# eth-cscs/conflux

Measured on NVIDIA B200. Metric: LU GFLOP/s (FP64, (2/3)N^3), higher is better.
Workload: dtype f64

## Files before the change

### conflux_b200/_lib.py

```python
import ctypes
import os

_HERE = os.path.dirname(os.path.abspath(__file__))
LIB_PATH = os.path.join(_HERE, "libconflux_b200.so")
_lib = None

c_double_p = ctypes.POINTER(ctypes.c_double)
c_int_p = ctypes.POINTER(ctypes.c_int)


class ConfluxError(RuntimeError):
    pass


SYMBOLS = [
    "cflx_last_error", "cflx_version", "cflx_device_count", "cflx_get_unique_id", "cflx_comm_create",
    "cflx_comm_barrier", "cflx_comm_destroy", "cflx_host_alloc", "cflx_host_free", "cflx_auto_grid", "cflx_lu_dims", "cflx_init_matrix_host",
    "cflx_lu_create", "cflx_lu_info", "cflx_lu_set_local", "cflx_lu_queue_next_local", "cflx_lu_factor", "cflx_lu_get_factors",
    "cflx_lu_get_permutation", "cflx_lu_residual", "cflx_lu_validate", "cflx_lu_solve", "cflx_lu_launch_count", "cflx_lu_uses_tcgen05", "cflx_lu_set_profiling", "cflx_lu_phase_ms", "cflx_lu_timeline",
    "cflx_lu_set_kernel_timing", "cflx_lu_trailing_stats", "cflx_lu_destroy", "cflx_chol_auto_grid", "cflx_chol_auto_tile", "cflx_chol_dims", "cflx_chol_init_matrix_host",
    "cflx_chol_create", "cflx_chol_info", "cflx_chol_set_local", "cflx_chol_factor", "cflx_chol_get_local", "cflx_chol_validate",
    "cflx_chol_launch_count", "cflx_chol_destroy", "cflx_dbg_gemm_tn", "cflx_dbg_panel", "cflx_dbg_trsm", "cflx_dbg_trsm_left_upper", "cflx_dbg_potrf_tile", "cflx_dbg_push_pivots", "cflx_dbg_ozaki_gemm", "cflx_dbg_umma_peak", "cflx_dbg_last_panel_cycles", "cflx_dbg_fp64_peak", "cflx_dbg_fp64_peak_ex",
]


def _preload_nccl():
    import sys
    for d in sys.path:
        cand = os.path.join(d, "nvidia", "nccl", "lib", "libnccl.so.2")
        if os.path.exists(cand):
            try:
                ctypes.CDLL(cand, mode=ctypes.RTLD_GLOBAL)
                return cand
            except OSError:
                pass
    return None


def lib():
    global _lib
    if _lib is None:
        if not os.path.exists(LIB_PATH):
            raise ConfluxError(
                f"{LIB_PATH} is missing: build it with `python -c 'import __graft_entry__ as g; g.build()'` "
                "(conflux_b200 has no CPU fallback)")
        _preload_nccl()
        L = ctypes.CDLL(LIB_PATH)
        L.cflx_last_error.restype = ctypes.c_char_p
        L.cflx_version.restype = ctypes.c_char_p
        L.cflx_comm_destroy.restype = None
        L.cflx_lu_destroy.restype = None
        L.cflx_comm_destroy.argtypes = [ctypes.c_void_p]
        L.cflx_lu_destroy.argtypes = [ctypes.c_void_p]
        L.cflx_comm_barrier.argtypes = [ctypes.c_void_p]
        L.cflx_comm_create.argtypes = [ctypes.c_int, ctypes.c_int, ctypes.c_void_p, ctypes.c_int,
                                       ctypes.POINTER(ctypes.c_void_p)]
        L.cflx_lu_create.argtypes = [ctypes.c_void_p] + [ctypes.c_int] * 6 + [ctypes.POINTER(ctypes.c_void_p)]
        L.cflx_host_alloc.argtypes = [ctypes.c_size_t, ctypes.POINTER(ctypes.c_void_p)]
        L.cflx_host_free.argtypes = [ctypes.c_void_p]
        L.cflx_lu_info.argtypes = [ctypes.c_void_p, c_int_p]
        L.cflx_lu_set_local.argtypes = [ctypes.c_void_p, ctypes.c_void_p]
        L.cflx_lu_queue_next_local.argtypes = [ctypes.c_void_p, ctypes.c_void_p]
        L.cflx_lu_factor.argtypes = [ctypes.c_void_p, c_double_p]
        L.cflx_lu_get_factors.argtypes = [ctypes.c_void_p, ctypes.c_void_p, ctypes.c_void_p]
        L.cflx_lu_get_permutation.argtypes = [ctypes.c_void_p, ctypes.c_void_p]
        L.cflx_lu_residual.argtypes = [ctypes.c_void_p, c_double_p]
        L.cflx_lu_validate.argtypes = [ctypes.c_void_p, c_double_p, c_double_p]
        L.cflx_lu_solve.argtypes = [ctypes.c_void_p, ctypes.c_int, ctypes.c_void_p, ctypes.c_void_p, c_double_p]
        L.cflx_lu_uses_tcgen05.argtypes = [ctypes.c_void_p]
        L.cflx_lu_launch_count.argtypes = [ctypes.c_void_p, ctypes.POINTER(ctypes.c_int64), ctypes.c_int]
        L.cflx_lu_set_profiling.argtypes = [ctypes.c_void_p, ctypes.c_int]
        L.cflx_lu_phase_ms.argtypes = [ctypes.c_void_p, c_double_p]
        L.cflx_lu_timeline.argtypes = [ctypes.c_void_p, ctypes.c_char_p, ctypes.c_int]
        L.cflx_lu_set_kernel_timing.argtypes = [ctypes.c_void_p, ctypes.c_int]
        L.cflx_lu_trailing_stats.argtypes = [ctypes.c_void_p, c_double_p, c_double_p]
        L.cflx_chol_destroy.restype = None
        L.cflx_chol_destroy.argtypes = [ctypes.c_void_p]
        L.cflx_chol_auto_grid.argtypes = [ctypes.c_int, ctypes.c_int, c_int_p]
        L.cflx_chol_auto_tile.argtypes = [ctypes.c_int] * 3
        L.cflx_chol_dims.argtypes = [ctypes.c_int] * 5 + [c_int_p]
        L.cflx_chol_init_matrix_host.argtypes = [ctypes.c_int] * 6 + [ctypes.c_void_p]
        L.cflx_chol_create.argtypes = [ctypes.c_void_p] + [ctypes.c_int] * 5 + [ctypes.POINTER(ctypes.c_void_p)]
        L.cflx_chol_info.argtypes = [ctypes.c_void_p, c_int_p]
        L.cflx_chol_set_local.argtypes = [ctypes.c_void_p, ctypes.c_void_p]
        L.cflx_chol_factor.argtypes = [ctypes.c_void_p, c_double_p]
        L.cflx_chol_get_local.argtypes = [ctypes.c_void_p, ctypes.c_void_p]
        L.cflx_chol_validate.argtypes = [ctypes.c_void_p, c_double_p, c_double_p]
        L.cflx_chol_launch_count.argtypes = [ctypes.c_void_p, ctypes.POINTER(ctypes.c_int64), ctypes.c_int]
        L.cflx_init_matrix_host.argtypes = [ctypes.c_int] * 8 + [ctypes.c_void_p]
        L.cflx_dbg_gemm_tn.argtypes = [ctypes.c_int] * 3 + [ctypes.c_void_p] * 3 + [ctypes.c_double] * 2 + [
            ctypes.c_void_p, ctypes.c_int, c_double_p]
        L.cflx_dbg_panel.argtypes = [ctypes.c_int, ctypes.c_int] + [ctypes.c_void_p] * 4 + [ctypes.c_int, c_double_p]
        L.cflx_dbg_trsm.argtypes = [ctypes.c_int, ctypes.c_int] + [ctypes.c_void_p] * 5
        L.cflx_dbg_trsm_left_upper.argtypes = [ctypes.c_int, ctypes.c_int] + [ctypes.c_void_p] * 3
        L.cflx_dbg_potrf_tile.argtypes = [ctypes.c_int, ctypes.c_int] + [ctypes.c_void_p] * 4
        L.cflx_dbg_push_pivots.argtypes = [ctypes.c_int, ctypes.c_int, ctypes.c_void_p, ctypes.c_int, ctypes.c_void_p, ctypes.c_int,
                                           ctypes.c_void_p, ctypes.c_void_p]
        L.cflx_dbg_ozaki_gemm.argtypes = [ctypes.c_int] * 3 + [ctypes.c_void_p] * 8 + [ctypes.c_int, c_double_p, c_double_p]
        L.cflx_dbg_umma_peak.argtypes = [ctypes.c_int, ctypes.c_int, c_double_p]
        L.cflx_dbg_fp64_peak.argtypes = [ctypes.c_int, c_double_p]
        L.cflx_dbg_fp64_peak_ex.argtypes = [ctypes.c_int, c_double_p, c_double_p]
        _lib = L
    return _lib


def check(rc, what=""):
    if rc != 0:
        msg = lib().cflx_last_error().decode(errors="replace")
        raise ConfluxError(f"{what} failed with status {rc}: {msg}")
```

### conflux_b200/csrc/dbg.cu

```cuda
#include <vector>

#include "../../include/conflux_b200.h"
#include "common.cuh"
#include "kernels.h"

using namespace cflx;

namespace {
struct DevBuf {
    void* p = nullptr;
    ~DevBuf() { cudaFree(p); }
    int alloc(size_t bytes) {
        CFLX_CUDA(cudaMalloc(&p, bytes + 4096));
        return CFLX_OK;
    }
    template <class T>
    T* as() { return (T*)p; }
};
int check_device() {
    int n = 0;
    if (cudaGetDeviceCount(&n) != cudaSuccess || n == 0) {
        cudaGetLastError();
        set_last_error("no CUDA device visible: conflux_b200 has no CPU fallback");
        return CFLX_ERR_NO_DEVICE;
    }
    return CFLX_OK;
}

__global__ void dmma_peak_kernel(double* out, int iters) {
    double c[16][2];
#pragma unroll
    for (int i = 0; i < 16; ++i) c[i][0] = c[i][1] = 0.0;
    double a = 1.0 + threadIdx.x * 1e-9, b = 1.0 - threadIdx.x * 1e-9;
    for (int it = 0; it < iters; ++it) {
#pragma unroll
        for (int i = 0; i < 16; ++i) dmma884(c[i][0], c[i][1], a, b);
    }
    double s = 0;
#pragma unroll
    for (int i = 0; i < 16; ++i) s += c[i][0] + c[i][1];
    out[blockIdx.x * blockDim.x + threadIdx.x] = s;
}
__global__ void dfma_peak_kernel(double* out, int iters) {
    double c[16];
#pragma unroll
    for (int i = 0; i < 16; ++i) c[i] = i;
    double a = 1.0 + threadIdx.x * 1e-9, b = 1e-9;
    for (int it = 0; it < iters; ++it) {
#pragma unroll
        for (int i = 0; i < 16; ++i) c[i] = fma(c[i], a, b);
    }
    double s = 0;
#pragma unroll
    for (int i = 0; i < 16; ++i) s += c[i];
    out[blockIdx.x * blockDim.x + threadIdx.x] = s;
}
}

static long long g_panel_cycles[8] = {0};

extern "C" {

int cflx_dbg_last_panel_cycles(long long* out8) {
    for (int i = 0; i < 8; ++i) out8[i] = g_panel_cycles[i];
    return CFLX_OK;
}

int cflx_dbg_fp64_peak_ex(int which, double* burst_out, double* sustained_out) {
    CFLX_TRY(check_device());
    int dev = 0, sms = 0;
    CFLX_CUDA(cudaGetDevice(&dev));
    CFLX_CUDA(cudaDeviceGetAttribute(&sms, cudaDevAttrMultiProcessorCount, dev));
    const int threads = 256, blocks = sms * 4;
    DevBuf out;
    CFLX_TRY(out.alloc(sizeof(double) * threads * blocks));
    cudaEvent_t e0, e1;
    CFLX_CUDA(cudaEventCreate(&e0));
    CFLX_CUDA(cudaEventCreate(&e1));
    auto run = [&](int iters, double* tf) -> int {
        CFLX_CUDA(cudaEventRecord(e0));
        if (which == 0) dmma_peak_kernel<<<blocks, threads>>>(out.as<double>(), iters);
        else dfma_peak_kernel<<<blocks, threads>>>(out.as<double>(), iters);
        CFLX_CUDA(cudaEventRecord(e1));
        CFLX_CUDA(cudaEventSynchronize(e1));
        float ms = 0;
        CFLX_CUDA(cudaEventElapsedTime(&ms, e0, e1));
        const double flop = which == 0 ? (double)blocks * (threads / 32) * iters * 16 * 512.0
                                       : (double)blocks * threads * iters * 16 * 2.0;
        *tf = flop / (ms * 1e-3) / 1e12;
        return CFLX_OK;
    };
    double burst = 0, tf = 0;
    for (int rep = 0; rep < 4; ++rep) {
        CFLX_TRY(run(1024, &tf));
        if (rep > 0 && tf > burst) burst = tf;
    }
    double sustained = 0;
    CFLX_TRY(run(262144, &sustained));
    cudaEventDestroy(e0);
    cudaEventDestroy(e1);
    if (burst_out) *burst_out = burst;
    if (sustained_out) *sustained_out = sustained;
    return CFLX_OK;
}
int cflx_dbg_fp64_peak(int which, double* tflops_out) { return cflx_dbg_fp64_peak_ex(which, tflops_out, nullptr); }

int cflx_dbg_gemm_tn(int M, int N, int K, const double* AT, const double* B, const double* C, double alpha, double beta,
                     double* D, int reps, double* ms_out) {
    CFLX_TRY(check_device());
    if (M <= 0 || N <= 0 || K <= 0) return CFLX_ERR_ARG;
    const int64_t ldat = round_up(M, 2), ldb = round_up(N, 2), ldc = ldb;
    DevBuf dA, dB, dC, dD;
    CFLX_TRY(dA.alloc(sizeof(double) * K * ldat));
    CFLX_TRY(dB.alloc(sizeof(double) * K * ldb));
    CFLX_TRY(dC.alloc(sizeof(double) * M * ldc));
    CFLX_TRY(dD.alloc(sizeof(double) * M * ldc));
    CFLX_CUDA(cudaMemset(dA.p, 0, sizeof(double) * K * ldat));
    CFLX_CUDA(cudaMemset(dB.p, 0, sizeof(double) * K * ldb));
    CFLX_CUDA(cudaMemcpy2D(dA.p, ldat * 8, AT, (size_t)M * 8, (size_t)M * 8, K, cudaMemcpyHostToDevice));
    CFLX_CUDA(cudaMemcpy2D(dB.p, ldb * 8, B, (size_t)N * 8, (size_t)N * 8, K, cudaMemcpyHostToDevice));
    if (C) CFLX_CUDA(cudaMemcpy2D(dC.p, ldc * 8, C, (size_t)N * 8, (size_t)N * 8, M, cudaMemcpyHostToDevice));
    else CFLX_CUDA(cudaMemset(dC.p, 0, sizeof(double) * M * ldc));
    GemmArgs g{};
    g.M = M; g.N = (int)ldb; g.K = K;
    g.AT = dA.as<double>(); g.ldat = ldat;
    g.B = dB.as<double>(); g.ldb = ldb;
    g.C = dC.as<double>(); g.ldc = ldc;
    g.D = dD.as<double>(); g.ldd = ldc;
    g.alpha = alpha; g.beta = beta;
    cudaEvent_t e0, e1;
    CFLX_CUDA(cudaEventCreate(&e0));
    CFLX_CUDA(cudaEventCreate(&e1));
    if (reps < 1) reps = 1;
    CFLX_TRY(launch_gemm_tn(g, 0));
    CFLX_CUDA(cudaEventRecord(e0));
    for (int r = 0; r < reps; ++r) CFLX_TRY(launch_gemm_tn(g, 0));
    CFLX_CUDA(cudaEventRecord(e1));
    CFLX_CUDA(cudaEventSynchronize(e1));
    float ms = 0;
    CFLX_CUDA(cudaEventElapsedTime(&ms, e0, e1));
    if (ms_out) *ms_out = ms / reps;
    cudaEventDestroy(e0);
    cudaEventDestroy(e1);
    if (D) CFLX_CUDA(cudaMemcpy2D(D, (size_t)N * 8, dD.p, ldc * 8, (size_t)N * 8, M, cudaMemcpyDeviceToHost));
    CFLX_CUDA(cudaDeviceSynchronize());
    return CFLX_OK;
}

int cflx_dbg_panel(int n, int v, const double* panel, int* perm_out, double* A00_out, double* LU_out, int reps,
                   double* ms_out) {
    CFLX_TRY(check_device());
    if (n < 0 || v <= 0) return CFLX_ERR_ARG;
    const int64_t ld = std::max<int64_t>(2, round_up(n, 2));
    std::vector<double> WT((size_t)v * ld, 0.0);
    for (int r = 0; r < n; ++r)
        for (int c = 0; c < v; ++c) WT[(size_t)c * ld + r] = panel[(size_t)r * v + c];
    DevBuf dW, dW0, dA00, dA00T, dperm;
    CFLX_TRY(dW.alloc(sizeof(double) * v * ld));
    CFLX_TRY(dW0.alloc(sizeof(double) * v * ld));
    CFLX_TRY(dA00.alloc(sizeof(double) * v * v));
    CFLX_TRY(dA00T.alloc(sizeof(double) * v * v));
    CFLX_TRY(dperm.alloc(sizeof(int) * 2 * v));
    CFLX_CUDA(cudaMemcpy(dW0.p, WT.data(), sizeof(double) * v * ld, cudaMemcpyHostToDevice));
    CFLX_CUDA(cudaMemset(dA00.p, 0, sizeof(double) * v * v));
    PanelWorkspace ws{};
    CFLX_TRY(panel_workspace_create(&ws));
    cudaEvent_t e0, e1;
    CFLX_CUDA(cudaEventCreate(&e0));
    CFLX_CUDA(cudaEventCreate(&e1));
    if (reps < 1) reps = 1;
    float total = 0;
    int nb = 0, rc = CFLX_OK;
    for (int r = 0; r < reps + 1 && rc == CFLX_OK; ++r) {
        cudaMemcpyAsync(dW.p, dW0.p, sizeof(double) * v * ld, cudaMemcpyDeviceToDevice, 0);
        cudaEventRecord(e0);
        rc = launch_panel_getrf_a00(dW.as<double>(), ld, n, v, dperm.as<int>(), dA00.as<double>(), &nb, &ws, 0);
        cudaEventRecord(e1);
        if (cudaEventSynchronize(e1) != cudaSuccess) rc = CFLX_ERR_CUDA;
        float ms = 0;
        cudaEventElapsedTime(&ms, e0, e1);
        if (r > 0) total += ms;
    }
    cudaEventDestroy(e0);
    cudaEventDestroy(e1);
    if (rc == CFLX_OK && n >= v)
        rc = launch_gather_a00(dW.as<double>(), ld, dperm.as<int>(), v, nb, dA00.as<double>(), dA00T.as<double>(), 0);
    cudaMemcpy(g_panel_cycles, ws.dbg, sizeof(g_panel_cycles), cudaMemcpyDeviceToHost);
    panel_workspace_destroy(&ws);
    if (rc != CFLX_OK) {
        if (rc == CFLX_ERR_CUDA) set_last_error("panel kernel failed: %s", cudaGetErrorString(cudaGetLastError()));
        return rc;
    }
    if (ms_out) *ms_out = total / reps;
    if (perm_out) CFLX_CUDA(cudaMemcpy(perm_out, dperm.p, sizeof(int) * v, cudaMemcpyDeviceToHost));
    if (A00_out) CFLX_CUDA(cudaMemcpy(A00_out, dA00.p, sizeof(double) * v * v, cudaMemcpyDeviceToHost));
    if (LU_out) {
        CFLX_CUDA(cudaMemcpy(WT.data(), dW.p, sizeof(double) * v * ld, cudaMemcpyDeviceToHost));
        for (int r = 0; r < n; ++r)
            for (int c = 0; c < v; ++c) LU_out[(size_t)r * v + c] = WT[(size_t)c * ld + r];
    }
    CFLX_CUDA(cudaDeviceSynchronize());
    return CFLX_OK;
}

int cflx_dbg_trsm(int n, int v, const double* A00, const double* B, double* X_out, const double* R, double* Y_out) {
    CFLX_TRY(check_device());
    if (n <= 0 || v <= 0 || v % 4 != 0) return CFLX_ERR_ARG;
    int nb = 0;
    for (int c : {128, 64, 32, 16, 8, 4})
        if (!nb && v % c == 0) nb = c;
    if (nb == 0) return CFLX_ERR_UNSUPPORTED;
    const int64_t ld = round_up(n, 2);
    std::vector<double> A00T((size_t)v * v), BT((size_t)v * ld, 0.0), RT((size_t)v * ld, 0.0);
    for (int i = 0; i < v; ++i)
        for (int j = 0; j < v; ++j) A00T[(size_t)j * v + i] = A00[(size_t)i * v + j];
    DevBuf dA, dAT, dUinv, dLinvT, dP, dL, dR, dU;
    CFLX_TRY(dA.alloc(8 * (size_t)v * v)); CFLX_TRY(dAT.alloc(8 * (size_t)v * v));
    CFLX_TRY(dUinv.alloc(8 * (size_t)v * v)); CFLX_TRY(dLinvT.alloc(8 * (size_t)v * v));
    CFLX_TRY(dP.alloc(8 * (size_t)v * ld)); CFLX_TRY(dL.alloc(8 * (size_t)v * ld));
    CFLX_TRY(dR.alloc(8 * (size_t)v * ld)); CFLX_TRY(dU.alloc(8 * (size_t)v * ld));
    CFLX_CUDA(cudaMemcpy(dA.p, A00, 8 * (size_t)v * v, cudaMemcpyHostToDevice));
    CFLX_CUDA(cudaMemcpy(dAT.p, A00T.data(), 8 * (size_t)v * v, cudaMemcpyHostToDevice));
    CFLX_TRY(launch_diag_inverses(dA.as<double>(), v, nb, dUinv.as<double>(), dLinvT.as<double>(), 0));
    if (B && X_out) {
        for (int r = 0; r < n; ++r)
            for (int c = 0; c < v; ++c) BT[(size_t)c * ld + r] = B[(size_t)r * v + c];
        CFLX_CUDA(cudaMemcpy(dP.p, BT.data(), 8 * (size_t)v * ld, cudaMemcpyHostToDevice));
        CFLX_CUDA(cudaMemset(dL.p, 0, 8 * (size_t)v * ld));
        CFLX_TRY(trsm_right_upper_T(dA.as<double>(), dUinv.as<double>(), v, nb, dP.as<double>(), dL.as<double>(), ld, n, 0));
        CFLX_CUDA(cudaMemcpy(BT.data(), dL.p, 8 * (size_t)v * ld, cudaMemcpyDeviceToHost));
        for (int r = 0; r < n; ++r)
            for (int c = 0; c < v; ++c) X_out[(size_t)r * v + c] = BT[(size_t)c * ld + r];
    }
    if (R && Y_out) {
        for (int i = 0; i < v; ++i)
            for (int c = 0; c < n; ++c) RT[(size_t)i * ld + c] = R[(size_t)i * n + c];
        CFLX_CUDA(cudaMemcpy(dR.p, RT.data(), 8 * (size_t)v * ld, cudaMemcpyHostToDevice));
        CFLX_CUDA(cudaMemset(dU.p, 0, 8 * (size_t)v * ld));
        CFLX_TRY(trsm_left_lower_unit(dAT.as<double>(), dLinvT.as<double>(), v, nb, dR.as<double>(), dU.as<double>(), ld,
                                      (int)ld, 0));
        CFLX_CUDA(cudaMemcpy(RT.data(), dU.p, 8 * (size_t)v * ld, cudaMemcpyDeviceToHost));
        for (int i = 0; i < v; ++i)
            for (int c = 0; c < n; ++c) Y_out[(size_t)i * n + c] = RT[(size_t)i * ld + c];
    }
    CFLX_CUDA(cudaDeviceSynchronize());
    return CFLX_OK;
}

int cflx_dbg_trsm_left_upper(int v, int n, const double* A00, const double* R, double* X_out) {
    CFLX_TRY(check_device());
    if (n <= 0 || v <= 0 || v % 4 != 0 || !A00 || !R || !X_out) return CFLX_ERR_ARG;
    int nb = 0;
    for (int c : {128, 64, 32, 16, 8, 4})
        if (!nb && v % c == 0) nb = c;
    if (nb == 0) return CFLX_ERR_UNSUPPORTED;
    const int64_t ld = round_up(n, 2);
    std::vector<double> A00T((size_t)v * v), RT((size_t)v * ld, 0.0);
    for (int i = 0; i < v; ++i)
        for (int j = 0; j < v; ++j) A00T[(size_t)j * v + i] = A00[(size_t)i * v + j];
    for (int i = 0; i < v; ++i)
        for (int c = 0; c < n; ++c) RT[(size_t)i * ld + c] = R[(size_t)i * n + c];
    DevBuf dA, dAT, dUinvT, dLinvT, dR, dX;
    CFLX_TRY(dA.alloc(8 * (size_t)v * v)); CFLX_TRY(dAT.alloc(8 * (size_t)v * v));
    CFLX_TRY(dUinvT.alloc(8 * (size_t)v * v)); CFLX_TRY(dLinvT.alloc(8 * (size_t)v * v));
    CFLX_TRY(dR.alloc(8 * (size_t)v * ld)); CFLX_TRY(dX.alloc(8 * (size_t)v * ld));
    CFLX_CUDA(cudaMemcpy(dA.p, A00, 8 * (size_t)v * v, cudaMemcpyHostToDevice));
    CFLX_CUDA(cudaMemcpy(dAT.p, A00T.data(), 8 * (size_t)v * v, cudaMemcpyHostToDevice));
    CFLX_CUDA(cudaMemcpy(dR.p, RT.data(), 8 * (size_t)v * ld, cudaMemcpyHostToDevice));
    CFLX_CUDA(cudaMemset(dX.p, 0, 8 * (size_t)v * ld));
    CFLX_TRY(launch_diag_inverses(dA.as<double>(), v, nb, dUinvT.as<double>(), dLinvT.as<double>(), 0, true));
    CFLX_TRY(trsm_left_upper(dAT.as<double>(), dUinvT.as<double>(), v, nb, dR.as<double>(), dX.as<double>(), ld, (int)ld, 0));
    CFLX_CUDA(cudaMemcpy(RT.data(), dX.p, 8 * (size_t)v * ld, cudaMemcpyDeviceToHost));
    for (int i = 0; i < v; ++i)
        for (int c = 0; c < n; ++c) X_out[(size_t)i * n + c] = RT[(size_t)i * ld + c];
    CFLX_CUDA(cudaDeviceSynchronize());
    return CFLX_OK;
}

int cflx_dbg_push_pivots(int n_rows, int n_cols, double* A_inout, int npiv, const int* pivot_rows, int fnpr, int* gri_out,
                         double* a01_out) {
    CFLX_TRY(check_device());
    if (n_rows <= 0 || n_cols <= 0 || (n_cols & 1) || npiv < 0 || npiv > n_rows - fnpr || fnpr < 0) return CFLX_ERR_ARG;
    if (npiv == 0) {
        if (gri_out) for (int i = 0; i < n_rows; ++i) gri_out[i] = i;
        return CFLX_OK;
    }
    const int v = npiv;
    DevBuf dA, dtmp, da01, dplan, dgp, dgri, dgrit, digri;
    CFLX_TRY(dA.alloc(8 * (size_t)n_rows * n_cols));
    CFLX_TRY(dtmp.alloc(8 * (size_t)v * n_cols));
    CFLX_TRY(da01.alloc(8 * (size_t)v * n_cols));
    CFLX_TRY(dplan.alloc(sizeof(int) * (6 * (size_t)v + 8 + n_rows)));
    CFLX_TRY(dgp.alloc(sizeof(int) * v));
    CFLX_TRY(dgri.alloc(sizeof(int) * n_rows));
    CFLX_TRY(dgrit.alloc(sizeof(int) * n_rows));
    CFLX_TRY(digri.alloc(sizeof(int) * n_rows));
    CFLX_CUDA(cudaMemcpy(dA.p, A_inout, 8 * (size_t)n_rows * n_cols, cudaMemcpyHostToDevice));
    CFLX_CUDA(cudaMemcpy(dgp.p, pivot_rows, sizeof(int) * v, cudaMemcpyHostToDevice));
    MovePlan plan{};
    int* pm = dplan.as<int>();
    plan.npiv = pm; plan.nel = pm + 4; pm += 8;
    plan.cur_piv = pm; pm += v;
    plan.order = pm; pm += v;
    plan.slot2piv = pm; pm += v;
    plan.early = pm; pm += v;
    plan.late = pm; pm += 2 * v;
    plan.rowsrc = pm;
    CFLX_TRY(launch_iota_gri(dgri.as<int>(), digri.as<int>(), n_rows, n_rows, 1, 0, 0));
    CFLX_TRY(launch_plan_moves(dgp.as<int>(), v, 1, 0, fnpr, n_rows, digri.as<int>(), plan, 0));
    CFLX_TRY(launch_push_phase1(dA.as<double>(), n_cols, n_cols, 0, plan, v, dtmp.as<double>(), da01.as<double>(), n_cols, 0, 0));
    CFLX_TRY(launch_push_phase2(dA.as<double>(), n_cols, n_cols, 0, plan, v, 0));
    CFLX_TRY(launch_push_phase3(dA.as<double>(), n_cols, n_cols, 0, fnpr, plan, v, dtmp.as<double>(), 0));
    CFLX_TRY(launch_update_gri(dgri.as<int>(), dgrit.as<int>(), digri.as<int>(), plan.rowsrc, fnpr, n_rows, n_rows, 1, 0));
    CFLX_CUDA(cudaMemcpy(A_inout, dA.p, 8 * (size_t)n_rows * n_cols, cudaMemcpyDeviceToHost));
    if (gri_out) CFLX_CUDA(cudaMemcpy(gri_out, dgri.p, sizeof(int) * n_rows, cudaMemcpyDeviceToHost));
    if (a01_out) CFLX_CUDA(cudaMemcpy(a01_out, da01.p, 8 * (size_t)v * n_cols, cudaMemcpyDeviceToHost));
    CFLX_CUDA(cudaDeviceSynchronize());
    return CFLX_OK;
}

int cflx_dbg_ozaki_gemm(int M, int N, int K, const double* AT, const double* B, const double* C, double* D,
                        signed char* planesA_out, signed char* planesB_out, int* ea_out, int* eb_out, int reps,
                        double* ms_out, double* split_ms_out) {
    CFLX_TRY(check_device());
    if (M <= 0 || N <= 0 || K <= 0 || (N & 1)) return CFLX_ERR_ARG;
    const int64_t ldat = round_up(M, 2), ldb = N, ldc = N;
    DevBuf dA, dB, dC, dC0;
    CFLX_TRY(dA.alloc(sizeof(double) * K * ldat));
    CFLX_TRY(dB.alloc(sizeof(double) * K * ldb));
    CFLX_TRY(dC.alloc(sizeof(double) * M * ldc));
    CFLX_TRY(dC0.alloc(sizeof(double) * M * ldc));
    CFLX_CUDA(cudaMemset(dA.p, 0, sizeof(double) * K * ldat));
    CFLX_CUDA(cudaMemcpy2D(dA.p, ldat * 8, AT, (size_t)M * 8, (size_t)M * 8, K, cudaMemcpyHostToDevice));
    CFLX_CUDA(cudaMemcpy(dB.p, B, sizeof(double) * K * ldb, cudaMemcpyHostToDevice));
    if (C) CFLX_CUDA(cudaMemcpy(dC0.p, C, sizeof(double) * M * ldc, cudaMemcpyHostToDevice));
    else CFLX_CUDA(cudaMemset(dC0.p, 0, sizeof(double) * M * ldc));
    OzakiWorkspace ws;
    int rc = ozaki_workspace_create(&ws, M, N, K);
    cudaEvent_t e0, e1, e2;
    cudaEventCreate(&e0);
    cudaEventCreate(&e1);
    cudaEventCreate(&e2);
    if (reps < 1) reps = 1;
    float ms = 0, ms_split = 0;
    for (int r = 0; r < reps + 1 && rc == CFLX_OK; ++r) {
        cudaMemcpyAsync(dC.p, dC0.p, sizeof(double) * M * ldc, cudaMemcpyDeviceToDevice, 0);
        cudaEventRecord(e0);
        rc = ozaki_split_a(&ws, dA.as<double>(), ldat, M, 0);
        if (!rc) rc = ozaki_split_b(&ws, dB.as<double>(), ldb, 0, N, 0);
        cudaEventRecord(e1);
        if (!rc) rc = launch_ozaki_gemm(&ws, M, N, 0, 0, dC.as<double>(), ldc, 0, 0);
        cudaEventRecord(e2);
        if (cudaEventSynchronize(e2) != cudaSuccess) {
            set_last_error("ozaki kernel failed: %s", cudaGetErrorString(cudaGetLastError()));
            rc = CFLX_ERR_CUDA;
        }
        float a = 0, b = 0;
        cudaEventElapsedTime(&a, e0, e1);
        cudaEventElapsedTime(&b, e1, e2);
        if (r > 0) {
            ms_split += a;
            ms += b;
        }
    }
    cudaEventDestroy(e0);
    cudaEventDestroy(e1);
    cudaEventDestroy(e2);
    if (rc == CFLX_OK) {
        if (D) cudaMemcpy(D, dC.p, sizeof(double) * M * ldc, cudaMemcpyDeviceToHost);
        for (int s = 0; s < 8; ++s) {
            if (planesA_out) cudaMemcpy(planesA_out + (size_t)s * M * K, ws.planesA + (size_t)s * ws.cap_a * K, (size_t)M * K, cudaMemcpyDeviceToHost);
            if (planesB_out) cudaMemcpy(planesB_out + (size_t)s * N * K, ws.planesB + (size_t)s * ws.cap_b * K, (size_t)N * K, cudaMemcpyDeviceToHost);
        }
        if (ea_out) cudaMemcpy(ea_out, ws.ea, sizeof(int) * M, cudaMemcpyDeviceToHost);
        if (eb_out) cudaMemcpy(eb_out, ws.eb, sizeof(int) * N, cudaMemcpyDeviceToHost);
        if (ws.dbg) {
            long long h[16];
            cudaMemcpy(h, ws.dbg, sizeof(h), cudaMemcpyDeviceToHost);
            fprintf(stderr, "[ozaki cycles, CTA 0] producer: wait emptyB %lld emptyA %lld total %lld | mma: wait fullA %lld fullB %lld tempty %lld "
                            "total %lld | epilogue: wait tfull %lld drain %lld rmw %lld total %lld\n",
                    h[0], h[1], h[3], h[4], h[5], h[6], h[7], h[8], h[9], h[10], h[11]);
        }
        if (cudaDeviceSynchronize() != cudaSuccess) rc = CFLX_ERR_CUDA;
    }
    ozaki_workspace_destroy(&ws);
    if (ms_out) *ms_out = ms / reps;
    if (split_ms_out) *split_ms_out = ms_split / reps;
    return rc;
}

int cflx_dbg_umma_peak(int which, int n, double* tmacs_out) {
    CFLX_TRY(check_device());
    if (!tmacs_out) return CFLX_ERR_ARG;
    return umma_peak_probe(n, which, tmacs_out);
}

}
```

### conflux_b200/csrc/kernels.h

```cpp
#pragma once
#include <cuda_runtime.h>

#include <cstdint>

namespace cflx {

struct GemmArgs {
    int M, N, K;
    const double* AT;
    int64_t ldat;
    const double* B;
    int64_t ldb;
    const double* C;
    int64_t ldc;
    double* D;
    int64_t ldd;
    double alpha, beta;
};
int gemm_tn_setup();
int launch_gemm_tn(const GemmArgs& g, cudaStream_t stream);

struct OzakiWorkspace {
    struct Maps;
    int8_t* planesA = nullptr;
    int8_t* planesB = nullptr;
    int* ea = nullptr;
    int* eb = nullptr;
    long long* dbg = nullptr;
    Maps* maps = nullptr;
    int K = 0, cap_a = 0, cap_b = 0, sms = 0;
};
int ozaki_workspace_create(OzakiWorkspace* ws, int max_rows, int max_cols, int K);
void ozaki_workspace_destroy(OzakiWorkspace* ws);
int ozaki_split_a(OzakiWorkspace* ws, const double* LT, int64_t ld, int n, cudaStream_t s);
int ozaki_split_b(OzakiWorkspace* ws, const double* U, int64_t ld, int col0, int n, cudaStream_t s);
int umma_peak_probe(int n, int use_f16, double* tmacs_out);
int launch_ozaki_gemm(OzakiWorkspace* ws, int M, int N, int row0, int col0, double* C, int64_t ldc, int max_ctas, cudaStream_t s);

struct PanelWorkspace {
    void* slot_hdr;
    void* slot_rows;
    long long* dbg;
    int epoch;
    int max_ctas;
    int cta_cap;
    unsigned* sk_flags;
    int* sk_ppos;
    unsigned* sk_ticket;
    unsigned sk_epoch, sk_ticket_count;
    int sk_enabled;
};
int panel_workspace_create(PanelWorkspace* ws);
void panel_workspace_destroy(PanelWorkspace* ws);
int launch_panel_getrf(double* W, int64_t ldw, int n, int v, int* perm_out, PanelWorkspace* ws, cudaStream_t stream);
int launch_panel_getrf_a00(double* W, int64_t ldw, int n, int v, int* perm_out, double* A00, int* nb_used,
                           PanelWorkspace* ws, cudaStream_t stream);

int launch_extract_panel_T(const double* A, int64_t lda, int64_t row0, int64_t col0, int n, int v, double* PT,
                           int64_t ldp, cudaStream_t stream);
int launch_store_panel_T(double* A, int64_t lda, int64_t row0, int64_t col0, int n, int v, const double* LT,
                         int64_t ldp, cudaStream_t stream);
int launch_gather_winners(const double* PT, int64_t ldp, const int* tags, int n_valid, const int* perm, int v,
                          double* out_vals, int64_t ldo, int* out_tags, int dst0, cudaStream_t stream);
int launch_gather_a00(const double* W, int64_t ldw, const int* perm, int v, int nb, double* A00, double* A00T,
                      cudaStream_t stream);

struct MovePlan {
    int* npiv;
    int* cur_piv;
    int* order;
    int* slot2piv;
    int* early;
    int* late;
    int* nel;
    int* rowsrc;
};
int launch_plan_moves(const int* gpivots, int v, int Px, int pi, int fnpr, int Ml, const int* igri, MovePlan plan,
                      cudaStream_t stream);
int launch_push_phase1(const double* A, int64_t lda, int ncols, int col_lo, MovePlan plan, int v, double* tmp,
                       double* a01raw, int64_t ld01, int c0, cudaStream_t stream);
int launch_push_phase2(double* A, int64_t lda, int ncols, int col_lo, MovePlan plan, int v, cudaStream_t stream);
int launch_push_phase3(double* A, int64_t lda, int ncols, int col_lo, int fnpr, MovePlan plan, int v,
                       const double* tmp, cudaStream_t stream);
int launch_update_gri(int* gri, int* gri_tmp, int* igri, const int* rowsrc, int fnpr, int Ml, int v, int Px,
                      cudaStream_t stream);
int launch_compact_panel(const double* PT, int64_t ldp, double* PT2, int64_t ldp2, const int* rowsrc, int fnpr_old,
                         const int* npiv, int Ml, int v, cudaStream_t stream);
int launch_store_u_rows(double* A, int64_t lda, int fnpr_old, MovePlan plan, const double* U, int64_t ldu, int c0,
                        int ncols, int v, cudaStream_t stream);
int launch_store_diag(double* A, int64_t lda, int fnpr_old, MovePlan plan, const double* A00, int loff, int v,
                      cudaStream_t stream);
int launch_split_factors(const double* F, int64_t ldf, int n, double* LT, double* U, cudaStream_t stream);
int launch_gather_perm_rows(const double* A, int64_t lda, const int* perm, int n, double* out, cudaStream_t stream);
int launch_sumsq(const double* X, int64_t count, double* out, cudaStream_t stream);
int launch_fill(double* p, int64_t n, double val, cudaStream_t stream);
int launch_iota_gri(int* gri, int* igri, int Ml, int v, int Px, int pi, cudaStream_t stream);
int launch_pack_bcast(const double* A00, const int* tags, int v, double* buf, cudaStream_t stream);
int launch_unpack_bcast(const double* buf, int v, double* A00, double* A00T, int* gpivots, cudaStream_t stream);
int launch_record_pivots(const int* gpivots, int v, int* hist, int k, cudaStream_t stream);

int launch_diag_inverses(const double* A00, int v, int nb, double* Uinv, double* LinvT, cudaStream_t stream,
                         bool u_transposed = false);
int trsm_right_upper_T(const double* A00, const double* Uinv, int v, int nb, double* PT, double* LT, int64_t ld,
                       int n, cudaStream_t stream);
int trsm_left_lower_unit(const double* A00T, const double* LinvT, int v, int nb, double* R, double* U, int64_t ld,
                         int n, cudaStream_t stream);
int trsm_left_upper(const double* A00T, const double* UinvT, int v, int nb, double* R, double* X, int64_t ld, int n,
                    cudaStream_t stream);

int launch_solve_update_skinny(const double* AT, int64_t ldat, int M, int K, const double* Y, int64_t ldy, int n,
                               double* W, int64_t ldw, cudaStream_t stream);
constexpr int SOLVE_SKINNY_MAX = 16;

}
```

### conflux_b200/csrc/lu.cu

```cuda
#include <algorithm>
#include <cmath>
#include <cstdarg>
#include <cstdlib>
#include <cstring>
#include <random>
#include <string>
#include <vector>

#include <nvtx3/nvToolsExt.h>

#include "lu_state.h"

namespace cflx {
static thread_local char g_err[1024] = "";
void set_last_error(const char* fmt, ...) {
    va_list ap;
    va_start(ap, fmt);
    vsnprintf(g_err, sizeof(g_err), fmt, ap);
    va_end(ap);
}
}

using namespace cflx;

namespace {
int flipbit(int n, int k) { return n ^ (1 << k); }
int butterfly_pair(int pi, int r, int Px) {
    int src = flipbit(pi, r);
    if (src >= Px) {
        if (r == 0) src = pi;
        else {
            src = flipbit(src, r - 1);
            if (src >= Px) src = Px - 1;
        }
    }
    return src;
}
#include "init_tables.inc"
bool fixed_input_matrix(int n, std::vector<double>* out) {
    for (const InitTable& t : kInitTables) {
        if (t.n != n) continue;
        out->clear();
        out->reserve((size_t)n * n);
        if (t.kind == 0) {
            for (const char* p = t.text; *p; ++p) out->push_back((double)(*p - '0'));
        } else {
            const char* p = t.text;
            while (*p) {
                char* e = nullptr;
                out->push_back(std::strtod(p, &e));
                p = (*e == ',') ? e + 1 : e;
            }
        }
        return out->size() == (size_t)n * n;
    }
    return false;
}
int pick_nb(int v) {
    static int cap = -1;
    if (cap < 0) {
        const char* e = getenv("CFLX_TRSM_NB");
        cap = e ? atoi(e) : 128;
    }
    for (int nb : {128, 64, 32, 16, 8, 4})
        if (nb <= cap && v % nb == 0) return nb;
    return 0;
}
}

namespace cflx {
int make_sub(cflx_comm* c, int color, int key, int size, SubComm* out) {
    out->size = size;
    out->rank = key;
    out->c = nullptr;
    if (c->world_size == 1) return CFLX_OK;
    CFLX_NCCL(ncclCommSplit(c->world, color, key, &out->c, nullptr));
    int r = -1, s = -1;
    CFLX_NCCL(ncclCommUserRank(out->c, &r));
    CFLX_NCCL(ncclCommCount(out->c, &s));
    if (r != key || s != size) {
        set_last_error("sub-communicator mismatch: rank %d/%d expected %d/%d", r, s, key, size);
        return CFLX_ERR_NCCL;
    }
    return CFLX_OK;
}
int grid_barrier(cflx_comm* c) {
    if (c->world_size > 1)
        CFLX_NCCL(ncclAllReduce(c->d_scratch, c->d_scratch, 1, ncclDouble, ncclSum, c->world, c->stream));
    CFLX_CUDA(cudaStreamSynchronize(c->stream));
    return CFLX_OK;
}
}

namespace {
struct PhaseTimer {
    cflx_lu* lu;
    int rg;
    cudaStream_t st;
    cudaEvent_t a = nullptr, b = nullptr;
    int ev = -1;
    PhaseTimer(cflx_lu* l, int region, cudaStream_t stream) : lu(l), rg(region), st(stream) {
        nvtxRangePushA(region_name(rg));
        if (lu->prof_mode == 1) {
            cudaEventCreate(&a);
            cudaEventCreate(&b);
            cudaEventRecord(a, st);
        } else if (lu->prof_mode == 2) {
            ev = (int)lu->tl_recs.size() * 2;
            while ((int)lu->tl_pool.size() < ev + 2) {
                cudaEvent_t e;
                cudaEventCreate(&e);
                lu->tl_pool.push_back(e);
            }
            lu->tl_recs.push_back({rg, st == lu->comm->stream ? 0 : 1, ev});
            cudaEventRecord(lu->tl_pool[ev], st);
        }
    }
    ~PhaseTimer() {
        if (lu->prof_mode == 1) {
            cudaEventRecord(b, st);
            cudaEventSynchronize(b);
            float ms = 0;
            cudaEventElapsedTime(&ms, a, b);
            lu->phase_ms[region_phase(rg)] += ms;
            lu->region_ms[st == lu->comm->stream ? 0 : 1][rg] += ms;
            lu->region_cnt[st == lu->comm->stream ? 0 : 1][rg]++;
            cudaEventDestroy(a);
            cudaEventDestroy(b);
        } else if (lu->prof_mode == 2) {
            cudaEventRecord(lu->tl_pool[ev + 1], st);
        }
        nvtxRangePop();
    }
};

int tournament_exchange(cflx_lu* lu, int r, int my_half, cudaStream_t s) {
    const int v = lu->v, Px = lu->Px, pi = lu->pi;
    const int src = butterfly_pair(pi, r, Px);
    const int other = 1 - my_half;
    const size_t hv = (size_t)v * v;
    double* mine = lu->candH + my_half * hv;
    double* recv = lu->candH + other * hv;
    int* mine_t = lu->tagsH + my_half * v;
    int* recv_t = lu->tagsH + other * v;
    const bool self = (src == pi);
    if (self) {
        CFLX_CUDA(cudaMemcpyAsync(recv, mine, hv * sizeof(double), cudaMemcpyDeviceToDevice, s));
        CFLX_CUDA(cudaMemcpyAsync(recv_t, mine_t, v * sizeof(int), cudaMemcpyDeviceToDevice, s));
    }
    bool any = !self;
    for (int ppi = 0; ppi < Px && !any; ++ppi) any = (ppi != pi && butterfly_pair(ppi, r, Px) == pi);
    if (!any) return CFLX_OK;
    CFLX_NCCL(ncclGroupStart());
    for (int ppi = 0; ppi < Px; ++ppi) {
        if (ppi == pi || butterfly_pair(ppi, r, Px) != pi) continue;
        const bool mutual = (!self && ppi == src);
        const double* sv = mutual ? mine : lu->candH + hv;
        const int* st = mutual ? mine_t : lu->tagsH + v;
        CFLX_NCCL(ncclSend(sv, hv, ncclDouble, ppi, lu->i_comm.c, s));
        CFLX_NCCL(ncclSend(st, v, ncclInt, ppi, lu->i_comm.c, s));
    }
    if (!self) {
        CFLX_NCCL(ncclRecv(recv, hv, ncclDouble, src, lu->i_comm.c, s));
        CFLX_NCCL(ncclRecv(recv_t, v, ncclInt, src, lu->i_comm.c, s));
    }
    CFLX_NCCL(ncclGroupEnd());
    return CFLX_OK;
}

__global__ void stack_kernel(const double* __restrict__ candH, const int* __restrict__ tagsH, int v, double* __restrict__ S,
                             double* __restrict__ W2, int* __restrict__ tagsS) {
    const int64_t e = (int64_t)blockIdx.x * blockDim.x + threadIdx.x;
    const int64_t tot = (int64_t)2 * v * v;
    if (e < tot) {
        const int c = (int)(e / (2 * v)), hi = (int)(e % (2 * v));
        const int h = hi / v, i = hi % v;
        const double x = candH[(size_t)h * v * v + (size_t)c * v + i];
        S[e] = x;
        W2[e] = x;
    }
    if (e < 2 * v) tagsS[e] = tagsH[e];
}
int panel_phase(cflx_lu* lu, int k, int fnpr, cudaStream_t s) {
    const int v = lu->v, Px = lu->Px, Py = lu->Py, Pz = lu->Pz, Ml = lu->Ml, Nl = lu->Nl;
    const int pi = lu->pi, pj = lu->pj, pk = lu->pk;
    const int loff = (k / Py) * v, pjk = k % Py;
    if (pj != pjk) return CFLX_OK;
    double* A00 = lu->A00 + (size_t)(k & 1) * v * v;
    double* A00T = lu->A00T + (size_t)(k & 1) * v * v;
    const int n_old = Ml - fnpr;
    const int64_t ldk = std::max<int64_t>(2, round_up(n_old, 2));
    int nR = 0;
    while ((1 << nR) < Px) ++nR;
    {
        PhaseTimer t(lu, RG_step0_copy, s);
        CFLX_TRY(launch_extract_panel_T(lu->A11, Nl, fnpr, loff, n_old, v, lu->PT, ldk, s));
        lu->launches++;
    }
    if (Pz > 1 && n_old > 0) {
        PhaseTimer t(lu, RG_step0_reduce, s);
        CFLX_NCCL(ncclReduce(lu->PT, lu->PT, (size_t)v * ldk, ncclDouble, ncclSum, 0, lu->k_comm.c, s));
    }
    if (pk != 0) return CFLX_OK;
    int my_half = 0;
    {
        PhaseTimer t(lu, RG_step1_A10copy, s);
        CFLX_CUDA(cudaMemcpyAsync(lu->W, lu->PT, (size_t)v * ldk * sizeof(double), cudaMemcpyDeviceToDevice, s));
    }
    {
        PhaseTimer t(lu, RG_step1_lup, s);
        int nb_used = 0;
        if (nR == 0) {
            CFLX_TRY(launch_panel_getrf_a00(lu->W, ldk, n_old, v, lu->perm, A00, &nb_used, &lu->pws, s));
            CFLX_TRY(launch_gather_a00(lu->W, ldk, lu->perm, v, nb_used, A00, A00T, s));
            lu->launches += 2;
        } else {
            CFLX_TRY(launch_panel_getrf(lu->W, ldk, n_old, v, lu->perm, &lu->pws, s));
            lu->launches++;
        }
    }
    {
        PhaseTimer t(lu, RG_step1_rowpermute, s);
        int first_partner = flipbit(pi, 0);
        if (first_partner > Px - 1) first_partner = Px - 1;
        my_half = first_partner < pi ? 1 : 0;
        CFLX_TRY(launch_gather_winners(lu->PT, ldk, lu->gri + fnpr, n_old, lu->perm, v,
                                       lu->candH + (size_t)my_half * v * v, v, lu->tagsH + my_half * v, 0, s));
        lu->launches++;
    }
    PhaseTimer t(lu, RG_step1_pivoting, s);
    for (int r = 0; r < nR; ++r) {
        CFLX_TRY(tournament_exchange(lu, r, my_half, s));
        const int64_t tot = (int64_t)2 * v * v;
        stack_kernel<<<(unsigned)((tot + 255) / 256), 256, 0, s>>>(lu->candH, lu->tagsH, v, lu->S, lu->W2, lu->tagsS);
        CFLX_CUDA(cudaGetLastError());
        const bool last = (r == nR - 1);
        int nb_used = 0;
        if (last) {
            CFLX_TRY(launch_panel_getrf_a00(lu->W2, 2 * v, 2 * v, v, lu->perm, A00, &nb_used, &lu->pws, s));
            CFLX_TRY(launch_gather_a00(lu->W2, 2 * v, lu->perm, v, nb_used, A00, A00T, s));
            lu->launches++;
            my_half = 0;
        } else {
            CFLX_TRY(launch_panel_getrf(lu->W2, 2 * v, 2 * v, v, lu->perm, &lu->pws, s));
            my_half = butterfly_pair(pi, r + 1, Px) < pi ? 1 : 0;
        }
        CFLX_TRY(launch_gather_winners(lu->S, 2 * v, lu->tagsS, 2 * v, lu->perm, v, lu->candH + (size_t)my_half * v * v,
                                       v, lu->tagsH + my_half * v, 0, s));
        lu->launches += 3;
    }
    return CFLX_OK;
}

int ozaki_planes_a(cflx_lu* lu, int n_act, int64_t ld2, cudaStream_t s) {
    if (!lu->use_ozaki || n_act <= 0) return CFLX_OK;
    PhaseTimer t(lu, RG_step6_dgemm, s);
    lu->launches++;
    return ozaki_split_a(&lu->oz, lu->LT + (int64_t)lu->pk * lu->nlayr * ld2, ld2, n_act, s);
}
int ozaki_planes_b(cflx_lu* lu, int col0, int n, int64_t ldu, cudaStream_t s) {
    if (!lu->use_ozaki || n <= 0) return CFLX_OK;
    PhaseTimer t(lu, RG_step6_dgemm, s);
    lu->launches++;
    return ozaki_split_b(&lu->oz, lu->U + (int64_t)lu->pk * lu->nlayr * ldu, ldu, col0, n, s);
}

int trailing_gemm(cflx_lu* lu, int k, int part, int fnpr, int n_act, int col_lo, int ncols, int64_t ld2, int64_t ldu,
                  int u_col_off, cudaStream_t s, int max_ctas = 0) {
    if (n_act <= 0 || ncols <= 0) return CFLX_OK;
    PhaseTimer t(lu, RG_step6_dgemm, s);
    GemmArgs g{};
    g.M = n_act;
    g.N = ncols;
    g.K = lu->nlayr;
    g.AT = lu->LT + (int64_t)lu->pk * lu->nlayr * ld2;
    g.ldat = ld2;
    g.B = lu->U + (int64_t)lu->pk * lu->nlayr * ldu + u_col_off;
    g.ldb = ldu;
    g.C = lu->A11 + (int64_t)fnpr * lu->Nl + col_lo;
    g.ldc = lu->Nl;
    g.D = lu->A11 + (int64_t)fnpr * lu->Nl + col_lo;
    g.ldd = lu->Nl;
    g.alpha = -1.0;
    g.beta = 1.0;
    const int e = 4 * k + 2 * part;
    if (lu->time_gemm) CFLX_CUDA(cudaEventRecord(lu->ev[e], s));
    if (lu->use_ozaki) CFLX_TRY(launch_ozaki_gemm(&lu->oz, g.M, g.N, 0, u_col_off, g.D, g.ldd, max_ctas, s));
    else CFLX_TRY(launch_gemm_tn(g, s));
    if (lu->time_gemm) CFLX_CUDA(cudaEventRecord(lu->ev[e + 1], s));
    lu->ev_used[e / 2] = lu->time_gemm;
    lu->gemm_flops += 2.0 * g.M * (double)g.N * g.K;
    lu->launches++;
    return CFLX_OK;
}

int finish_step(cflx_lu* lu, int k, int& fnpr) {
    cudaStream_t s = lu->comm->stream;
    const int v = lu->v, Px = lu->Px, Py = lu->Py, Pz = lu->Pz, Ml = lu->Ml, Nl = lu->Nl;
    const int pi = lu->pi, pj = lu->pj, pk = lu->pk;
    const int loff = (k / Py) * v, pjk = k % Py, pik = k % Px;
    const bool on_col = (pj == pjk), on_row = (pi == pik), layer0 = (pk == 0);
    const int c0 = loff + (pj <= pjk ? v : 0);
    const int ncols = Nl - c0;
    const int fnpr_old = fnpr;
    const int n_old = Ml - fnpr_old;
    const int64_t ldk = std::max<int64_t>(2, round_up(n_old, 2));
    int nR = 0;
    while ((1 << nR) < Px) ++nR;
    double* A00 = lu->A00 + (size_t)(k & 1) * v * v;
    double* A00T = lu->A00T + (size_t)(k & 1) * v * v;
    {
        PhaseTimer t(lu, RG_step1_A00Buff_bcast, s);
        if (lu->P > 1) {
            const int root = (pik * Py + pjk) * Pz;
            if (lu->rank == root) {
                CFLX_TRY(launch_pack_bcast(A00, lu->tagsH, v, lu->bcast, s));
                lu->launches++;
            }
            CFLX_NCCL(ncclBroadcast(lu->bcast, lu->bcast, (size_t)v * v + v, ncclDouble, root, lu->comm->world, s));
            CFLX_TRY(launch_unpack_bcast(lu->bcast, v, A00, A00T, lu->gpivots, s));
            lu->launches++;
        } else {
            CFLX_CUDA(cudaMemcpyAsync(lu->gpivots, lu->tagsH, v * sizeof(int), cudaMemcpyDeviceToDevice, s));
        }
        CFLX_TRY(launch_record_pivots(lu->gpivots, v, lu->hist, k, s));
        lu->launches++;
    }
    {
        PhaseTimer t(lu, RG_step2_pushingpivots, s);
        CFLX_TRY(launch_plan_moves(lu->gpivots, v, Px, pi, fnpr_old, Ml, lu->igri, lu->plan, s));
        lu->launches++;
        if (Px > 1) {
            CFLX_CUDA(cudaMemcpyAsync(lu->h_npiv, lu->plan.npiv, sizeof(int), cudaMemcpyDeviceToHost, s));
            CFLX_CUDA(cudaEventRecord(lu->ev_npiv, s));
        }
        const int col_lo = layer0 ? 0 : loff;
        const int64_t ldu0 = std::max(2, ncols);
        CFLX_TRY(launch_push_phase1(lu->A11, Nl, Nl, col_lo, lu->plan, v, lu->tmp, ncols > 0 ? lu->A01raw : nullptr, ldu0, c0,
                                    s));
        CFLX_TRY(launch_push_phase2(lu->A11, Nl, Nl, col_lo, lu->plan, v, s));
        CFLX_TRY(launch_push_phase3(lu->A11, Nl, Nl, col_lo, fnpr_old, lu->plan, v, lu->tmp, s));
        CFLX_TRY(launch_update_gri(lu->gri, lu->gri_tmp, lu->igri, lu->plan.rowsrc, fnpr_old, Ml, v, Px, s));
        lu->launches += 5;
    }
    const int64_t ldu = std::max(2, ncols);
    const bool fused_l = (nR == 0);
    if (ncols > 0 && Px * Pz > 1) {
        PhaseTimer t(lu, RG_step2_reduce, s);
        CFLX_NCCL(ncclReduce(lu->A01raw, lu->A01raw, (size_t)v * ldu, ncclDouble, ncclSum, pik * Pz, lu->ik_comm.c, s));
    }
    if (layer0 && ((on_col && !fused_l) || on_row)) {
        PhaseTimer t(lu, RG_step5_dtrsm, s);
        CFLX_TRY(launch_diag_inverses(A00, v, lu->nb, lu->Uinv, lu->LinvT, s));
        lu->launches++;
    }
    const bool split_u = (lu->P == 1) && (k + 1 < lu->Nt) && ncols > v;
    const int ncols_a = split_u ? v : ncols;
    if (on_row && layer0 && ncols > 0) {
        PhaseTimer t(lu, RG_step5_dtrsm, s);
        CFLX_TRY(trsm_left_lower_unit(A00T, lu->LinvT, v, lu->nb, lu->A01raw, lu->U, ldu, ncols_a, s));
        lu->launches += 2 * (v / lu->nb) - 1;
    }
    if (Px * Pz > 1 && ncols > 0) {
        PhaseTimer t(lu, RG_step5_comm, s);
        CFLX_NCCL(ncclBroadcast(lu->U, lu->U, (size_t)v * ldu, ncclDouble, pik * Pz, lu->ik_comm.c, s));
    }
    auto store_factors = [&]() -> int {
        if (!layer0) return CFLX_OK;
        PhaseTimer t(lu, RG_storingresults, s);
        if (ncols > 0) {
            CFLX_TRY(launch_store_u_rows(lu->A11, Nl, fnpr_old, lu->plan, lu->U, ldu, c0, ncols, v, s));
            lu->launches++;
        }
        if (on_col) {
            CFLX_TRY(launch_store_diag(lu->A11, Nl, fnpr_old, lu->plan, A00, loff, v, s));
            lu->launches++;
        }
        return CFLX_OK;
    };
    if (!split_u) CFLX_TRY(store_factors());
    int npiv = v;
    if (Px > 1) {
        CFLX_CUDA(cudaEventSynchronize(lu->ev_npiv));
        npiv = *lu->h_npiv;
    }
    if (npiv < 0 || npiv > v || fnpr_old + npiv > Ml) {
        set_last_error("step %d: inconsistent pivot count %d (fnpr %d, Ml %d)", k, npiv, fnpr_old, Ml);
        return CFLX_ERR_STATE;
    }
    fnpr = fnpr_old + npiv;
    const int n_act = Ml - fnpr;
    const int64_t ld2 = std::max<int64_t>(2, round_up(n_act, 2));
    if (on_col && layer0 && n_act > 0) {
        {
            PhaseTimer t(lu, RG_step4_reshuffling, s);
            CFLX_TRY(launch_compact_panel(fused_l ? lu->W : lu->PT, ldk, fused_l ? lu->LT : lu->PT2, ld2, lu->plan.rowsrc,
                                          fnpr_old, lu->plan.npiv, Ml, v, s));
            lu->launches++;
        }
        if (!fused_l) {
            PhaseTimer t(lu, RG_step4_dtrsm, s);
            CFLX_TRY(trsm_right_upper_T(A00, lu->Uinv, v, lu->nb, lu->PT2, lu->LT, ld2, n_act, s));
            lu->launches += 2 * (v / lu->nb) - 1;
        }
        PhaseTimer t(lu, RG_storingresults, s);
        CFLX_TRY(launch_store_panel_T(lu->A11, Nl, fnpr, loff, n_act, v, lu->LT, ld2, s));
        lu->launches++;
    }
    if (Py * Pz > 1 && n_act > 0) {
        PhaseTimer t(lu, RG_step4_comm, s);
        CFLX_NCCL(ncclBroadcast(lu->LT, lu->LT, (size_t)v * ld2, ncclDouble, pjk * Pz, lu->jk_comm.c, s));
    }
    const bool next_col = (k + 1 < lu->Nt) && (pj == (k + 1) % Py);
    CFLX_TRY(ozaki_planes_a(lu, n_act, ld2, s));
    if (n_act > 0) CFLX_TRY(ozaki_planes_b(lu, 0, split_u ? std::min(v, ncols) : ncols, ldu, s));
    if (next_col) {
        const int w = std::min(v, ncols);
        CFLX_TRY(trailing_gemm(lu, k, 0, fnpr, n_act, c0, w, ld2, ldu, 0, s));
        cudaStream_t side = (lu->prof_mode == 1) ? nullptr : lu->side;
        cudaStream_t sp = side ? side : s;
        if (side) {
            CFLX_CUDA(cudaEventRecord(lu->ev_fork, s));
            CFLX_CUDA(cudaStreamWaitEvent(sp, lu->ev_fork, 0));
        }
        CFLX_TRY(panel_phase(lu, k + 1, fnpr, sp));
        if (side) CFLX_CUDA(cudaEventRecord(lu->ev_join, sp));
        if (split_u) {
            PhaseTimer t(lu, RG_step5_dtrsm, s);
            CFLX_TRY(trsm_left_lower_unit(A00T, lu->LinvT, v, lu->nb, lu->A01raw + v, lu->U + v, ldu, ncols - v, s));
            lu->launches += 2 * (v / lu->nb) - 1;
        }
        if (split_u) CFLX_TRY(store_factors());
        if (split_u && n_act > 0) CFLX_TRY(ozaki_planes_b(lu, w, ncols - w, ldu, s));
        const int leave = (side && lu->use_ozaki) ? lu->pws.cta_cap : 0;
        CFLX_TRY(trailing_gemm(lu, k, 1, fnpr, n_act, c0 + w, ncols - w, ld2, ldu, w, s, leave > 0 ? lu->oz.sms - leave : 0));
        if (side) CFLX_CUDA(cudaStreamWaitEvent(s, lu->ev_join, 0));
    } else {
        CFLX_TRY(trailing_gemm(lu, k, 0, fnpr, n_act, c0, ncols, ld2, ldu, 0, s));
    }
    return CFLX_OK;
}

void free_lu(cflx_lu* lu) {
    if (!lu) return;
    cudaSetDevice(lu->comm->device);
    double* dbl[] = {lu->A0, lu->A11, lu->PT, lu->PT2, lu->W, lu->LT, lu->A01raw, lu->U, lu->tmp, lu->A00, lu->A00T,
                     lu->Uinv, lu->LinvT, lu->candH, lu->S, lu->W2, lu->bcast, lu->Cbuf, lu->xbuf};
    for (double* p : dbl) cudaFree(p);
    int* ints[] = {lu->gri, lu->gri_tmp, lu->igri, lu->perm, lu->gpivots, lu->tagsH, lu->tagsS, lu->hist, lu->plan_mem,
                   lu->idx_buf};
    for (int* p : ints) cudaFree(p);
    if (lu->h_npiv) cudaFreeHost(lu->h_npiv);
    if (lu->pws.slot_hdr) panel_workspace_destroy(&lu->pws);
    if (lu->use_ozaki) ozaki_workspace_destroy(&lu->oz);
    for (auto& e : lu->ev) cudaEventDestroy(e);
    for (auto& e : lu->tl_pool) cudaEventDestroy(e);
    if (lu->side) cudaStreamDestroy(lu->side);
    if (lu->ev_fork) cudaEventDestroy(lu->ev_fork);
    if (lu->ev_join) cudaEventDestroy(lu->ev_join);
    if (lu->ev_npiv) cudaEventDestroy(lu->ev_npiv);
    if (lu->copy) cudaStreamDestroy(lu->copy);
    if (lu->ev_a0_read) cudaEventDestroy(lu->ev_a0_read);
    if (lu->ev_upload) cudaEventDestroy(lu->ev_upload);
    solve_state_free(&lu->sv);
    for (SubComm* sc : {&lu->k_comm, &lu->i_comm, &lu->jk_comm, &lu->ik_comm})
        if (sc->c) ncclCommDestroy(sc->c);
    delete lu;
}
}

extern "C" {

const char* cflx_last_error(void) { return g_err; }
const char* cflx_version(void) { return "conflux_b200 0.1 (sm_100a)"; }

int cflx_device_count(int* count) {
    int n = 0;
    cudaError_t e = cudaGetDeviceCount(&n);
    if (e != cudaSuccess) {
        n = 0;
        cudaGetLastError();
    }
    *count = n;
    return CFLX_OK;
}

int cflx_get_unique_id(void* id_out) {
    static_assert(sizeof(ncclUniqueId) == CFLX_UNIQUE_ID_BYTES, "unique id size");
    ncclUniqueId id;
    CFLX_NCCL(ncclGetUniqueId(&id));
    std::memcpy(id_out, &id, sizeof(id));
    return CFLX_OK;
}

int cflx_comm_create(int world_size, int world_rank, const void* unique_id, int device, cflx_comm** out) {
    if (!out || world_size < 1 || world_rank < 0 || world_rank >= world_size) return CFLX_ERR_ARG;
    int ndev = 0;
    cflx_device_count(&ndev);
    if (ndev == 0) {
        set_last_error("no CUDA device visible: conflux_b200 has no CPU fallback");
        return CFLX_ERR_NO_DEVICE;
    }
    if (device < 0 || device >= ndev) {
        set_last_error("device %d out of range (%d visible)", device, ndev);
        return CFLX_ERR_ARG;
    }
    CFLX_CUDA(cudaSetDevice(device));
    auto* c = new cflx_comm;
    c->world_size = world_size;
    c->world_rank = world_rank;
    c->device = device;
    CFLX_CUDA(cudaStreamCreateWithFlags(&c->stream, cudaStreamNonBlocking));
    CFLX_CUDA(cudaMalloc((void**)&c->d_scratch, sizeof(double)));
    CFLX_CUDA(cudaMemset(c->d_scratch, 0, sizeof(double)));
    if (world_size > 1) {
        if (!unique_id) {
            set_last_error("unique_id required for world_size > 1");
            return CFLX_ERR_ARG;
        }
        ncclUniqueId id;
        std::memcpy(&id, unique_id, sizeof(id));
        CFLX_NCCL(ncclCommInitRank(&c->world, world_size, id, world_rank));
    }
    *out = c;
    return CFLX_OK;
}

int cflx_comm_barrier(cflx_comm* c) {
    if (!c) return CFLX_ERR_ARG;
    CFLX_CUDA(cudaSetDevice(c->device));
    return grid_barrier(c);
}

void cflx_comm_destroy(cflx_comm* c) {
    if (!c) return;
    cudaSetDevice(c->device);
    if (c->world) ncclCommDestroy(c->world);
    if (c->stream) cudaStreamDestroy(c->stream);
    cudaFree(c->d_scratch);
    delete c;
}

int cflx_auto_grid(int M, int N, int P, int* Px, int* Py, int* Pz) {
    if (M <= 0 || N <= 0 || P <= 0) return CFLX_ERR_ARG;
    const double ratio = 1.0 * std::max(M, N) / std::min(M, N);
    const int p1 = (int)std::cbrt(P / ratio);
    const int psq = (int)std::sqrt(P / ratio);
    const int phs = (int)std::sqrt(P / (2 * ratio));
    if (P == psq * psq) {
        *Px = psq; *Py = psq; *Pz = 1;
        return CFLX_OK;
    }
    if (phs * phs == P / 2) {
        *Px = phs; *Py = phs; *Pz = 2;
        return CFLX_OK;
    }
    int d[3] = {p1, (int)(ratio * p1), 0};
    d[2] = P / (d[0] * d[1]);
    std::sort(d, d + 3, [](int a, int b) { return a > b; });
    *Px = d[0]; *Py = d[1]; *Pz = d[2];
    return CFLX_OK;
}

int cflx_lu_dims(int M, int N, int v, int Px, int Py, int Pz, int* o) {
    if (M <= 0 || N <= 0 || v <= 0 || Px <= 0 || Py <= 0 || Pz <= 0 || !o) return CFLX_ERR_ARG;
    const int tx = (int)std::ceil((double)M / (v * Px)), ty = (int)std::ceil((double)N / (v * Py));
    const int Mp = v * Px * tx, Np = v * Py * ty;
    const int Nt = (int)std::ceil((double)Np / v), Mt = (int)std::ceil((double)Mp / v);
    o[0] = Mp; o[1] = Np;
    o[2] = (int)std::ceil((double)Mt / Px) * v;
    o[3] = (int)std::ceil((double)Nt / Py) * v;
    o[4] = Nt; o[5] = (v + Pz - 1) / Pz; o[6] = Mt; o[7] = Px * Py * Pz;
    return CFLX_OK;
}

int cflx_init_matrix_host(int M, int N, int v, int Px, int Py, int Pz, int rank, int seed, double* out) {
    int d[8];
    CFLX_TRY(cflx_lu_dims(M, N, v, Px, Py, Pz, d));
    const int Ml = d[2], Nl = d[3];
    if (rank < 0 || rank >= d[7] || !out) return CFLX_ERR_ARG;
    std::fill(out, out + (size_t)Ml * Nl, 0.0);
    if (rank % Pz != 0) return CFLX_OK;
    if (d[0] == d[1]) {
        std::vector<double> tab;
        if (fixed_input_matrix(d[0], &tab)) {
            const int n = d[0], pi = rank / (Py * Pz), pj = (rank / Pz) % Py;
            for (int lr = 0; lr < Ml; ++lr) {
                const int gi = ((lr / v) * Px + pi) * v + lr % v;
                for (int lc = 0; lc < Nl; ++lc) {
                    const int gj = ((lc / v) * Py + pj) * v + lc % v;
                    out[(size_t)lr * Nl + lc] = tab[(size_t)gi * n + gj];
                }
            }
            return CFLX_OK;
        }
    }
    std::mt19937_64 eng((unsigned long long)(seed + rank));
    std::uniform_real_distribution<double> dist;
    for (int lti = 0; lti < Ml / v; ++lti)
        for (int ltj = 0; ltj < Nl / v; ++ltj)
            for (int li = 0; li < v; ++li)
                for (int lj = 0; lj < v; ++lj) out[(size_t)(lti * v + li) * Nl + ltj * v + lj] = 5 + dist(eng);
    return CFLX_OK;
}

int cflx_lu_create(cflx_comm* c, int M, int N, int v, int Px, int Py, int Pz, cflx_lu** out) {
    if (!c || !out || M <= 0 || N <= 0 || v <= 0) return CFLX_ERR_ARG;
    CFLX_CUDA(cudaSetDevice(c->device));
    if (Px <= 0 || Py <= 0 || Pz <= 0) CFLX_TRY(cflx_auto_grid(M, N, c->world_size, &Px, &Py, &Pz));
    if (Px != Py) {
        set_last_error("grid %dx%dx%d: the CONFLUX LU path requires Px == Py (SURVEY.md fact 6)", Px, Py, Pz);
        return CFLX_ERR_UNSUPPORTED;
    }
    if (Px * Py * Pz != c->world_size) {
        set_last_error("grid %dx%dx%d does not match the %d ranks of the communicator", Px, Py, Pz, c->world_size);
        return CFLX_ERR_ARG;
    }
    if (v % 4 != 0 || v % Pz != 0 || (v / Pz) % 4 != 0 || pick_nb(v) == 0) {
        set_last_error("tile size v=%d unsupported: need v %% 4 == 0 and (v / Pz) %% 4 == 0", v);
        return CFLX_ERR_UNSUPPORTED;
    }
    int d[8];
    CFLX_TRY(cflx_lu_dims(M, N, v, Px, Py, Pz, d));
    auto* lu = new cflx_lu;
    lu->comm = c;
    lu->M = d[0]; lu->N = d[1]; lu->Ml = d[2]; lu->Nl = d[3]; lu->Nt = d[4]; lu->nlayr = d[5]; lu->Mt = d[6]; lu->P = d[7];
    lu->v = v; lu->Px = Px; lu->Py = Py; lu->Pz = Pz;
    lu->rank = c->world_rank;
    lu->pi = lu->rank / (Py * Pz);
    lu->pj = (lu->rank / Pz) % Py;
    lu->pk = lu->rank % Pz;
    lu->nb = pick_nb(v);
    if (lu->M != lu->N) {
        set_last_error("only square matrices are supported (the miniapp passes M = N)");
        delete lu;
        return CFLX_ERR_UNSUPPORTED;
    }
    int rc = CFLX_OK;
    auto fail = [&](int code) {
        free_lu(lu);
        return code;
    };
    if ((rc = make_sub(c, lu->pi * Py + lu->pj, lu->pk, Pz, &lu->k_comm))) return fail(rc);
    if ((rc = make_sub(c, lu->pj * Pz + lu->pk, lu->pi, Px, &lu->i_comm))) return fail(rc);
    if ((rc = make_sub(c, lu->pi, lu->pj * Pz + lu->pk, Py * Pz, &lu->jk_comm))) return fail(rc);
    if ((rc = make_sub(c, lu->pj, lu->pi * Pz + lu->pk, Px * Pz, &lu->ik_comm))) return fail(rc);

    const size_t loc = (size_t)lu->Ml * lu->Nl;
    const int64_t ldp = round_up(lu->Ml, 2) + 2;
    lu->ldp_max = ldp;
    const size_t pan = (size_t)v * ldp, upan = (size_t)v * (lu->Nl + 2), vv = (size_t)v * v;
#define ALLOC(ptr, n) if ((rc = dmalloc(&(ptr), (n)))) return fail(rc)
    ALLOC(lu->A0, loc); ALLOC(lu->A11, loc);
    ALLOC(lu->PT, pan); ALLOC(lu->PT2, pan); ALLOC(lu->W, pan); ALLOC(lu->LT, pan);
    ALLOC(lu->A01raw, upan); ALLOC(lu->U, upan); ALLOC(lu->tmp, (size_t)v * lu->Nl);
    ALLOC(lu->A00, 2 * vv); ALLOC(lu->A00T, 2 * vv); ALLOC(lu->Uinv, vv); ALLOC(lu->LinvT, vv);
    ALLOC(lu->candH, 2 * vv); ALLOC(lu->S, 2 * vv); ALLOC(lu->W2, 2 * vv); ALLOC(lu->bcast, vv + v);
    ALLOC(lu->gri, lu->Ml); ALLOC(lu->gri_tmp, lu->Ml); ALLOC(lu->igri, lu->Ml); ALLOC(lu->perm, 2 * v);
    ALLOC(lu->gpivots, v); ALLOC(lu->tagsH, 2 * v); ALLOC(lu->tagsS, 2 * v); ALLOC(lu->hist, lu->M);
    ALLOC(lu->plan_mem, 6 * (size_t)v + 8 + lu->Ml);
#undef ALLOC
    int* pm = lu->plan_mem;
    lu->plan.npiv = pm; lu->plan.nel = pm + 4; pm += 8;
    lu->plan.cur_piv = pm; pm += v;
    lu->plan.order = pm; pm += v;
    lu->plan.slot2piv = pm; pm += v;
    lu->plan.early = pm; pm += v;
    lu->plan.late = pm; pm += v;
    pm += v;
    lu->plan.rowsrc = pm;
    if (cudaMallocHost((void**)&lu->h_npiv, sizeof(int)) != cudaSuccess) return fail(CFLX_ERR_CUDA);
    if (cudaEventCreateWithFlags(&lu->ev_npiv, cudaEventDisableTiming) != cudaSuccess) return fail(CFLX_ERR_CUDA);
    if ((rc = panel_workspace_create(&lu->pws))) return fail(rc);
    if ((rc = gemm_tn_setup())) return fail(rc);
    {
        const char* e = getenv("CFLX_GEMM");
        const bool want = !(e && !strcmp(e, "dmma"));
        if (want && lu->nlayr % 128 == 0 && lu->nlayr <= 512) {
            if ((rc = ozaki_workspace_create(&lu->oz, lu->Ml, lu->Nl, lu->nlayr))) return fail(rc);
            lu->use_ozaki = true;
        }
    }
    lu->h_hist.assign(lu->M, -1);
    {
        const char* e = getenv("CFLX_LOOKAHEAD");
        const char* em = getenv("CFLX_LOOKAHEAD_MULTI");
        const bool want = (e ? atoi(e) != 0 : true) && (lu->P == 1 || !em || atoi(em) != 0);
        if (want) {
            int lo = 0, hi = 0;
            cudaDeviceGetStreamPriorityRange(&lo, &hi);
            if (cudaStreamCreateWithPriority(&lu->side, cudaStreamNonBlocking, hi) != cudaSuccess) return fail(CFLX_ERR_CUDA);
            if (cudaEventCreateWithFlags(&lu->ev_fork, cudaEventDisableTiming) != cudaSuccess) return fail(CFLX_ERR_CUDA);
            if (cudaEventCreateWithFlags(&lu->ev_join, cudaEventDisableTiming) != cudaSuccess) return fail(CFLX_ERR_CUDA);
            const char* c = getenv("CFLX_PANEL_CTAS");
            lu->pws.cta_cap = c ? atoi(c) : (lu->P == 1 ? 32 : (lu->Px == 1 ? 48 : 64));
        }
    }
    cudaMemsetAsync(lu->PT, 0, pan * sizeof(double), c->stream);
    cudaMemsetAsync(lu->PT2, 0, pan * sizeof(double), c->stream);
    cudaMemsetAsync(lu->LT, 0, pan * sizeof(double), c->stream);
    cudaMemsetAsync(lu->W, 0, pan * sizeof(double), c->stream);
    cudaMemsetAsync(lu->A01raw, 0, upan * sizeof(double), c->stream);
    cudaMemsetAsync(lu->U, 0, upan * sizeof(double), c->stream);
    cudaMemsetAsync(lu->A0, 0, loc * sizeof(double), c->stream);
    if (cudaStreamSynchronize(c->stream) != cudaSuccess) return fail(CFLX_ERR_CUDA);
    *out = lu;
    return CFLX_OK;
}

int cflx_lu_info(const cflx_lu* lu, int* o) {
    if (!lu || !o) return CFLX_ERR_ARG;
    const int vals[16] = {lu->M, lu->N, lu->Ml, lu->Nl, lu->Nt, lu->nlayr, lu->P, lu->Px, lu->Py, lu->Pz, lu->pi, lu->pj,
                          lu->pk, lu->rank, lu->v, 0};
    std::memcpy(o, vals, sizeof(vals));
    return CFLX_OK;
}

int cflx_lu_set_local(cflx_lu* lu, const double* host_local) {
    if (!lu || !host_local) return CFLX_ERR_ARG;
    CFLX_CUDA(cudaSetDevice(lu->comm->device));
    const size_t loc = (size_t)lu->Ml * lu->Nl;
    CFLX_CUDA(cudaMemcpyAsync(lu->A0, host_local, loc * sizeof(double), cudaMemcpyHostToDevice, lu->comm->stream));
    CFLX_CUDA(cudaStreamSynchronize(lu->comm->stream));
    lu->have_input = true;
    lu->factored = false;
    lu->sv.ready = false;
    lu->a0_is_next = false;
    lu->next_host = nullptr;
    return CFLX_OK;
}

int cflx_lu_queue_next_local(cflx_lu* lu, const double* host_next) {
    if (!lu || !host_next) return CFLX_ERR_ARG;
    if (!lu->have_input) {
        set_last_error("cflx_lu_queue_next_local needs a current input (cflx_lu_set_local) first");
        return CFLX_ERR_STATE;
    }
    CFLX_CUDA(cudaSetDevice(lu->comm->device));
    if (!lu->copy) {
        CFLX_CUDA(cudaStreamCreateWithFlags(&lu->copy, cudaStreamNonBlocking));
        CFLX_CUDA(cudaEventCreateWithFlags(&lu->ev_a0_read, cudaEventDisableTiming));
        CFLX_CUDA(cudaEventCreateWithFlags(&lu->ev_upload, cudaEventDisableTiming));
    }
    lu->next_host = host_next;
    return CFLX_OK;
}

int cflx_lu_factor(cflx_lu* lu, double* ms_out) {
    if (!lu) return CFLX_ERR_ARG;
    if (!lu->have_input) {
        set_last_error("cflx_lu_factor before cflx_lu_set_local");
        return CFLX_ERR_STATE;
    }
    lu->sv.ready = false;
    cflx_comm* c = lu->comm;
    cudaStream_t s = c->stream;
    CFLX_CUDA(cudaSetDevice(c->device));
    const size_t loc = (size_t)lu->Ml * lu->Nl;
    {
        PhaseTimer t(lu, RG_init, s);
        if (lu->a0_is_next) CFLX_CUDA(cudaStreamWaitEvent(s, lu->ev_upload, 0));
        CFLX_CUDA(cudaMemcpyAsync(lu->A11, lu->A0, loc * sizeof(double), cudaMemcpyDeviceToDevice, s));
    }
    lu->a0_is_next = false;
    if (lu->next_host) {
        CFLX_CUDA(cudaEventRecord(lu->ev_a0_read, s));
        CFLX_CUDA(cudaStreamWaitEvent(lu->copy, lu->ev_a0_read, 0));
        CFLX_CUDA(cudaMemcpyAsync(lu->A0, lu->next_host, loc * sizeof(double), cudaMemcpyHostToDevice, lu->copy));
        CFLX_CUDA(cudaEventRecord(lu->ev_upload, lu->copy));
        lu->next_host = nullptr;
        lu->a0_is_next = true;
    }
    CFLX_TRY(launch_iota_gri(lu->gri, lu->igri, lu->Ml, lu->v, lu->Px, lu->pi, s));
    for (double& x : lu->phase_ms) x = 0;
    for (int sd = 0; sd < 2; ++sd)
        for (int r = 0; r < RG_COUNT; ++r) lu->region_ms[sd][r] = 0, lu->region_cnt[sd][r] = 0;
    lu->tl_recs.clear();
    CFLX_TRY(grid_barrier(c));
    cudaEvent_t e0, e1;
    CFLX_CUDA(cudaEventCreate(&e0));
    CFLX_CUDA(cudaEventCreate(&e1));
    CFLX_CUDA(cudaEventRecord(e0, s));
    int fnpr = 0;
    lu->gemm_flops = 0;
    lu->gemm_ms = 0;
    if (lu->time_gemm && (int)lu->ev.size() < 4 * lu->Nt) {
        for (auto& e : lu->ev) cudaEventDestroy(e);
        lu->ev.assign(4 * lu->Nt, nullptr);
        for (auto& e : lu->ev) CFLX_CUDA(cudaEventCreate(&e));
    }
    lu->ev_used.assign(2 * lu->Nt, 0);
    {
        cudaStream_t side = (lu->prof_mode == 1) ? nullptr : lu->side;
        if (side) {
            CFLX_CUDA(cudaEventRecord(lu->ev_fork, s));
            CFLX_CUDA(cudaStreamWaitEvent(side, lu->ev_fork, 0));
        }
        int rc0 = panel_phase(lu, 0, 0, side ? side : s);
        if (rc0 != CFLX_OK) return rc0;
        if (side) {
            CFLX_CUDA(cudaEventRecord(lu->ev_join, side));
            CFLX_CUDA(cudaStreamWaitEvent(s, lu->ev_join, 0));
        }
    }
    for (int k = 0; k < lu->Nt; ++k) {
        int rc = finish_step(lu, k, fnpr);
        if (rc != CFLX_OK) {
            cudaEventDestroy(e0);
            cudaEventDestroy(e1);
            return rc;
        }
    }
    CFLX_CUDA(cudaEventRecord(e1, s));
    CFLX_CUDA(cudaEventSynchronize(e1));
    float ms = 0;
    CFLX_CUDA(cudaEventElapsedTime(&ms, e0, e1));
    cudaEventDestroy(e0);
    cudaEventDestroy(e1);
    CFLX_CUDA(cudaGetLastError());
    if (ms_out) *ms_out = ms;
    if (lu->prof_mode == 2) {
        if (lu->side) cudaStreamSynchronize(lu->side);
        for (const auto& r : lu->tl_recs) {
            float g = 0;
            if (cudaEventElapsedTime(&g, lu->tl_pool[r.ev], lu->tl_pool[r.ev + 1]) == cudaSuccess) {
                lu->region_ms[r.side][r.region] += g;
                lu->region_cnt[r.side][r.region]++;
                lu->phase_ms[region_phase(r.region)] += g;
            } else {
                cudaGetLastError();
            }
        }
    }
    if (lu->time_gemm) {
        for (int i = 0; i < 2 * lu->Nt; ++i) {
            if (!lu->ev_used[i]) continue;
            float g = 0;
            if (cudaEventElapsedTime(&g, lu->ev[2 * i], lu->ev[2 * i + 1]) == cudaSuccess) lu->gemm_ms += g;
            else cudaGetLastError();
        }
    }
    if (lu->a0_is_next) CFLX_CUDA(cudaStreamSynchronize(lu->copy));
    lu->factored = true;
    return CFLX_OK;
}

int cflx_lu_get_permutation(cflx_lu* lu, int* perm_out) {
    if (!lu || !perm_out) return CFLX_ERR_ARG;
    if (!lu->factored) {
        set_last_error("permutation requested before cflx_lu_factor");
        return CFLX_ERR_STATE;
    }
    CFLX_CUDA(cudaSetDevice(lu->comm->device));
    CFLX_CUDA(cudaMemcpyAsync(lu->h_hist.data(), lu->hist, sizeof(int) * lu->M, cudaMemcpyDeviceToHost, lu->comm->stream));
    CFLX_CUDA(cudaStreamSynchronize(lu->comm->stream));
    std::memcpy(perm_out, lu->h_hist.data(), sizeof(int) * lu->M);
    return CFLX_OK;
}

int cflx_lu_get_factors(cflx_lu* lu, double* C_host, int* perm_out) {
    if (!lu) return CFLX_ERR_ARG;
    if (!lu->factored) {
        set_last_error("factors requested before cflx_lu_factor");
        return CFLX_ERR_STATE;
    }
    cflx_comm* c = lu->comm;
    cudaStream_t s = c->stream;
    CFLX_CUDA(cudaSetDevice(c->device));
    std::vector<int> hist(lu->M);
    CFLX_TRY(cflx_lu_get_permutation(lu, hist.data()));
    if (perm_out) std::memcpy(perm_out, hist.data(), sizeof(int) * lu->M);
    if (lu->pk != 0) return CFLX_OK;
    const size_t loc = (size_t)lu->Ml * lu->Nl;
    if (!lu->Cbuf) CFLX_TRY(dmalloc(&lu->Cbuf, loc));
    CFLX_TRY(redistribute_pivoted_rows(lu, hist, true, lu->A11, lu->Cbuf));
    if (C_host) CFLX_CUDA(cudaMemcpyAsync(C_host, lu->Cbuf, loc * sizeof(double), cudaMemcpyDeviceToHost, s));
    CFLX_CUDA(cudaStreamSynchronize(s));
    return CFLX_OK;
}

int cflx_lu_validate(cflx_lu* lu, double* frob_abs_out, double* frob_rel_out) {
    if (!lu) return CFLX_ERR_ARG;
    if (!lu->factored) {
        set_last_error("residual requested before cflx_lu_factor");
        return CFLX_ERR_STATE;
    }
    if (lu->a0_is_next) {
        set_last_error("residual refused: the input buffer of the last run was handed to the queued next matrix");
        return CFLX_ERR_STATE;
    }
    CFLX_CUDA(cudaSetDevice(lu->comm->device));
    std::vector<int> hist(lu->M);
    CFLX_TRY(cflx_lu_get_permutation(lu, hist.data()));
    return lu_residual_grid(lu, hist, frob_abs_out, frob_rel_out);
}
int cflx_lu_residual(cflx_lu* lu, double* rel_out) {
    if (!rel_out) return CFLX_ERR_ARG;
    return cflx_lu_validate(lu, nullptr, rel_out);
}

int cflx_host_alloc(size_t bytes, void** out) {
    if (!out) return CFLX_ERR_ARG;
    int n = 0;
    cflx_device_count(&n);
    if (n == 0) {
        set_last_error("no CUDA device visible: conflux_b200 has no CPU fallback");
        return CFLX_ERR_NO_DEVICE;
    }
    CFLX_CUDA(cudaHostAlloc(out, bytes, cudaHostAllocPortable));
    return CFLX_OK;
}
int cflx_host_free(void* p) {
    if (p) CFLX_CUDA(cudaFreeHost(p));
    return CFLX_OK;
}

int cflx_lu_uses_tcgen05(const cflx_lu* lu) { return lu && lu->use_ozaki ? 1 : 0; }
int cflx_lu_launch_count(cflx_lu* lu, int64_t* count_out, int reset) {
    if (!lu || !count_out) return CFLX_ERR_ARG;
    *count_out = lu->launches;
    if (reset) lu->launches = 0;
    return CFLX_OK;
}
int cflx_lu_set_profiling(cflx_lu* lu, int mode) {
    if (!lu || mode < 0 || mode > 2) return CFLX_ERR_ARG;
    lu->prof_mode = mode;
    return CFLX_OK;
}
int cflx_lu_timeline(cflx_lu* lu, char* buf, int buf_len) {
    if (!lu) return CFLX_ERR_ARG;
    std::string o = "{";
    for (int sd = 0; sd < 2; ++sd) {
        o += sd ? ", \"side\": {" : "\"main\": {";
        bool first = true;
        for (int r = 0; r < RG_COUNT; ++r) {
            if (!lu->region_cnt[sd][r]) continue;
            char tmp[160];
            snprintf(tmp, sizeof(tmp), "%s\"%s\": [%.4f, %d]", first ? "" : ", ", region_name(r), lu->region_ms[sd][r], lu->region_cnt[sd][r]);
            o += tmp;
            first = false;
        }
        o += "}";
    }
    o += "}";
    if (!buf || buf_len <= (int)o.size()) return (int)o.size() + 1;
    std::memcpy(buf, o.c_str(), o.size() + 1);
    return CFLX_OK;
}
int cflx_lu_phase_ms(cflx_lu* lu, double* ms_out) {
    if (!lu || !ms_out) return CFLX_ERR_ARG;
    for (int i = 0; i < PH_COUNT; ++i) ms_out[i] = lu->phase_ms[i];
    return CFLX_OK;
}
int cflx_lu_set_kernel_timing(cflx_lu* lu, int enabled) {
    if (!lu) return CFLX_ERR_ARG;
    lu->time_gemm = enabled != 0;
    return CFLX_OK;
}
int cflx_lu_trailing_stats(cflx_lu* lu, double* ms_out, double* flops_out) {
    if (!lu || !ms_out || !flops_out) return CFLX_ERR_ARG;
    *ms_out = lu->gemm_ms;
    *flops_out = lu->gemm_flops;
    return CFLX_OK;
}
void cflx_lu_destroy(cflx_lu* lu) { free_lu(lu); }

}
```

### conflux_b200/csrc/lu_state.h

```cpp
#pragma once
#include <nccl.h>

#include <algorithm>
#include <vector>

#include "../../include/conflux_b200.h"
#include "common.cuh"
#include "kernels.h"

#define CFLX_NCCL(call)                                                                                    \
    do {                                                                                                   \
        ncclResult_t r__ = (call);                                                                         \
        if (r__ != ncclSuccess) {                                                                          \
            ::cflx::set_last_error("%s:%d: %s -> %s", __FILE__, __LINE__, #call, ncclGetErrorString(r__)); \
            return CFLX_ERR_NCCL;                                                                          \
        }                                                                                                  \
    } while (0)

struct cflx_comm {
    int world_size = 1, world_rank = 0, device = 0;
    ncclComm_t world = nullptr;
    cudaStream_t stream = nullptr;
    double* d_scratch = nullptr;
};

namespace cflx {
struct SubComm {
    ncclComm_t c = nullptr;
    int size = 1, rank = 0;
};

enum Phase { PH_PANEL = 0, PH_TOURN, PH_MOVES, PH_REDUCE, PH_TRSM, PH_GEMM, PH_STORE, PH_OTHER, PH_COUNT };

enum Region {
    RG_init = 0, RG_step0_copy, RG_step0_reduce, RG_step1_A10copy, RG_step1_lup, RG_step1_rowpermute, RG_step1_pivoting,
    RG_step1_A00Buff_bcast, RG_step2_pushingpivots, RG_step2_reduce, RG_step4_reshuffling, RG_step4_dtrsm, RG_step4_comm,
    RG_step5_dtrsm, RG_step5_comm, RG_step6_dgemm, RG_storingresults, RG_COUNT
};
inline const char* region_name(int r) {
    static const char* n[RG_COUNT] = {"init", "step0_copy", "step0_reduce", "step1_A10copy", "step1_lup", "step1_rowpermute",
                                      "step1_pivoting", "step1_A00Buff_bcast", "step2_pushingpivots", "step2_reduce",
                                      "step4_reshuffling", "step4_dtrsm", "step4_comm", "step5_dtrsm", "step5_comm",
                                      "step6_dgemm", "storingresults"};
    return n[r];
}
inline int region_phase(int r) {
    static const int p[RG_COUNT] = {PH_OTHER, PH_PANEL, PH_PANEL, PH_PANEL, PH_PANEL, PH_PANEL, PH_TOURN, PH_TOURN, PH_MOVES,
                                    PH_REDUCE, PH_MOVES, PH_TRSM, PH_REDUCE, PH_TRSM, PH_REDUCE, PH_GEMM, PH_STORE};
    return p[r];
}

template <class T>
inline int dmalloc(T** p, size_t n) {
    CFLX_CUDA(cudaMalloc((void**)p, std::max<size_t>(n, 1) * sizeof(T) + 4096));
    return CFLX_OK;
}
int make_sub(cflx_comm* c, int color, int key, int size, SubComm* out);
int grid_barrier(cflx_comm* c);

struct SolveState {
    bool ready = false;
    std::vector<int> hist;
    std::vector<int> diag_slot;
    double* CT = nullptr;
    double* diag = nullptr;
    double *W = nullptr, *X = nullptr, *B = nullptr, *stage = nullptr;
    int ldr_cap = 0;
};
}

struct cflx_lu {
    cflx_comm* comm = nullptr;
    int M = 0, N = 0, v = 0, Px = 1, Py = 1, Pz = 1, P = 1, Ml = 0, Nl = 0, Nt = 0, Mt = 0, nlayr = 0;
    int pi = 0, pj = 0, pk = 0, rank = 0, nb = 0;
    cflx::SubComm k_comm, i_comm, jk_comm, ik_comm;
    double *A0 = nullptr, *A11 = nullptr, *PT = nullptr, *PT2 = nullptr, *W = nullptr, *LT = nullptr, *A01raw = nullptr,
           *U = nullptr, *tmp = nullptr, *A00 = nullptr, *A00T = nullptr, *Uinv = nullptr, *LinvT = nullptr,
           *candH = nullptr, *S = nullptr, *W2 = nullptr, *bcast = nullptr, *Cbuf = nullptr, *xbuf = nullptr;
    int *gri = nullptr, *gri_tmp = nullptr, *igri = nullptr, *perm = nullptr, *gpivots = nullptr, *tagsH = nullptr,
        *tagsS = nullptr, *hist = nullptr, *plan_mem = nullptr, *idx_buf = nullptr;
    cflx::MovePlan plan{};
    cflx::PanelWorkspace pws{};
    cflx::OzakiWorkspace oz{};
    bool use_ozaki = false;
    int64_t ldp_max = 0;
    int* h_npiv = nullptr;
    std::vector<int> h_hist;
    bool have_input = false, factored = false, time_gemm = false;
    const double* next_host = nullptr;
    bool a0_is_next = false;
    cudaStream_t copy = nullptr;
    cudaEvent_t ev_a0_read = nullptr, ev_upload = nullptr;
    double gemm_ms = 0, gemm_flops = 0;
    int64_t launches = 0;
    double phase_ms[cflx::PH_COUNT] = {0};
    struct TlRec { int region, side, ev; };
    std::vector<cudaEvent_t> tl_pool;
    std::vector<TlRec> tl_recs;
    double region_ms[2][cflx::RG_COUNT] = {{0}};
    int region_cnt[2][cflx::RG_COUNT] = {{0}};
    int prof_mode = 0;
    std::vector<cudaEvent_t> ev;
    std::vector<char> ev_used;
    cudaStream_t side = nullptr;
    cudaEvent_t ev_fork = nullptr, ev_join = nullptr, ev_npiv = nullptr;
    cflx::SolveState sv;
};

namespace cflx {
int redistribute_pivoted_rows(cflx_lu* lu, const std::vector<int>& hist, bool factors, const double* src, double* dst);
int redistribute_pivoted_rows(cflx_lu* lu, const std::vector<int>& hist, bool factors, const double* src, double* dst,
                              int ncols, int64_t ld, double* stage);
int lu_residual_grid(cflx_lu* lu, const std::vector<int>& hist, double* abs_out, double* rel_out);
void solve_state_free(SolveState* sv);
}
```

### conflux_b200/csrc/panel.cu

```cuda
#include <cooperative_groups.h>

#include <climits>
#include <cstdlib>

#include "common.cuh"
#include "kernels.h"

namespace cflx {

namespace {
constexpr int PT_THREADS = 256;
constexpr int PT_WARPS = PT_THREADS / 32;
constexpr int MAXG = 148;
constexpr int RPT_LIMIT = 8;

struct PanelArgs {
    double* W;
    int64_t ldw;
    int n, v, nsteps;
    int R, Rpad, G;
    int* perm_out;
    double* A00;
    uint2* slot_hdr;
    uint2* slot_rows;
    int epoch_base;
    int spec;
    long long* dbg;
};

__device__ __forceinline__ void st_ll(uint2* p, unsigned data, unsigned epoch) {
    asm volatile("st.volatile.global.v2.u32 [%0], {%1, %2};" ::"l"(p), "r"(data), "r"(epoch) : "memory");
}
__device__ __forceinline__ uint4 ld_ll2(const uint2* p) {
    uint4 v;
    asm volatile("ld.volatile.global.v4.u32 {%0, %1, %2, %3}, [%4];" : "=r"(v.x), "=r"(v.y), "=r"(v.z), "=r"(v.w) : "l"(p) : "memory");
    return v;
}

constexpr int CS_MAX = 8;
__device__ __forceinline__ void st_ll_dsmem(const uint2* local_slot, unsigned peer, unsigned data, unsigned epoch) {
    unsigned remote;
    asm volatile("mapa.shared::cluster.u32 %0, %1, %2;" : "=r"(remote) : "r"(smem_u32(local_slot)), "r"(peer));
    asm volatile("st.shared::cluster.v2.u32 [%0], {%1, %2};" ::"r"(remote), "r"(data), "r"(epoch) : "memory");
}
__device__ __forceinline__ uint4 ld_ll2_smem(const uint2* p) {
    uint4 v;
    asm volatile("ld.volatile.shared.v4.u32 {%0, %1, %2, %3}, [%4];" : "=r"(v.x), "=r"(v.y), "=r"(v.z), "=r"(v.w) : "r"(smem_u32(p)) : "memory");
    return v;
}
__device__ __forceinline__ void cluster_sync_all() {
    asm volatile("barrier.cluster.arrive.release.aligned;" ::: "memory");
    asm volatile("barrier.cluster.wait.acquire.aligned;" ::: "memory");
}

struct Cand {
    unsigned long long key;
    int pos;
    int row;
};

__device__ __forceinline__ Cand warp_argmax(Cand c) {
    const unsigned hi = (unsigned)(c.key >> 32), lo = (unsigned)c.key;
    const unsigned m1 = __reduce_max_sync(0xffffffffu, hi);
    bool in = (hi == m1);
    const unsigned m2 = __reduce_max_sync(0xffffffffu, in ? lo : 0u);
    in = in && (lo == m2);
    const unsigned m3 = __reduce_min_sync(0xffffffffu, in ? (unsigned)c.pos : (unsigned)INT_MAX);
    const unsigned ballot = __ballot_sync(0xffffffffu, in && (unsigned)c.pos == m3);
    const int src = __ffs(ballot) - 1;
    Cand r;
    r.key = ((unsigned long long)m1 << 32) | m2;
    r.pos = (int)m3;
    r.row = __shfl_sync(0xffffffffu, c.row, src);
    return r;
}
__device__ __forceinline__ bool better(const Cand& a, const Cand& b) {
    return a.key > b.key || (a.key == b.key && a.pos < b.pos);
}
__device__ __forceinline__ Cand block_argmax(Cand c, unsigned long long* red_key, int* red_pos, int* red_row, int& rb) {
    Cand w = warp_argmax(c);
    const int warp = threadIdx.x >> 5;
    const int o = rb * PT_WARPS;
    rb ^= 1;
    if ((threadIdx.x & 31) == 0) {
        red_key[o + warp] = w.key;
        red_pos[o + warp] = w.pos;
        red_row[o + warp] = w.row;
    }
    __syncthreads();
    Cand best{red_key[o], red_pos[o], red_row[o]};
#pragma unroll
    for (int i = 1; i < PT_WARPS; ++i) {
        Cand x{red_key[o + i], red_pos[o + i], red_row[o + i]};
        if (better(x, best)) best = x;
    }
    return best;
}

template <int NB, int RPT_MAX, bool DSM>
__global__ void __launch_bounds__(PT_THREADS, 1) panel_getrf_kernel(PanelArgs p) {
    extern __shared__ __align__(16) unsigned char smem_raw[];
    double* Ab = reinterpret_cast<double*>(smem_raw);
    double* U12 = Ab + (size_t)NB * p.Rpad;
    double* LU11 = U12 + (size_t)NB * p.v;
    double* prow = LU11 + NB * (NB + 1);
    double* crow = prow + 2 * NB;
    unsigned long long* red_key = reinterpret_cast<unsigned long long*>(crow + 2 * 32 * NB);
    int* red_pos = reinterpret_cast<int*>(red_key + 2 * PT_WARPS);
    int* red_row = red_pos + 2 * PT_WARPS;
    int* pivrow_blk = red_row + 2 * PT_WARPS;
    int* win_sh = pivrow_blk + NB;
    uint2* cs_hdr = reinterpret_cast<uint2*>(win_sh + 4);
    uint2* cs_row = cs_hdr + 2 * CS_MAX * 4;
    unsigned char* s_act = reinterpret_cast<unsigned char*>(cs_row + 2 * CS_MAX * 2 * NB);
    int rb = 0;

    const int t = threadIdx.x;
    const int cta = blockIdx.x;
    const int row_base = cta * p.R;
    const int Rloc = max(0, min(p.R, p.n - row_base));
    const int Rpad = p.Rpad, v = p.v;
    double* __restrict__ W = p.W;
    const int64_t ldw = p.ldw;

    long long tm[8] = {0, 0, 0, 0, 0, 0, 0, 0};
    long long t0 = clock64(), t1;
#define TICK(i)            \
    t1 = clock64();        \
    tm[i] += t1 - t0;      \
    t0 = t1;
    int pos[RPT_MAX];
    bool active[RPT_MAX];
    int pib[RPT_MAX];
#pragma unroll
    for (int q = 0; q < RPT_MAX; ++q) {
        const int lr = t + q * PT_THREADS;
        pos[q] = row_base + lr;
        active[q] = lr < Rloc;
        pib[q] = -1;
    }
    for (int lr = t; lr < Rpad; lr += PT_THREADS) s_act[lr] = lr < Rloc ? 1 : 0;
    if constexpr (DSM) {
        for (int e = t; e < 2 * CS_MAX * (4 + 2 * NB); e += PT_THREADS) cs_hdr[e] = make_uint2(0u, 0u);
        __syncthreads();
        cluster_sync_all();
    }

    for (int jb = 0; jb < p.nsteps; jb += NB) {
        const int nbc = min(NB, v - jb);
        const int nsb = min(nbc, p.nsteps - jb);
        for (int e = t; e < nbc * Rpad; e += PT_THREADS) {
            const int c = e / Rpad, lr = e - c * Rpad;
            if (lr < Rloc) Ab[e] = W[(int64_t)(jb + c) * ldw + row_base + lr];
        }
        __syncthreads();
        TICK(5)

        auto local_candidate = [&](int col) -> Cand {
            Cand c{0ull, INT_MAX, -1};
#pragma unroll
            for (int q = 0; q < RPT_MAX; ++q) {
                const int lr = t + q * PT_THREADS;
                if (active[q]) {
                    Cand o{(unsigned long long)__double_as_longlong(fabs(Ab[col * Rpad + lr])), pos[q], row_base + lr};
                    if (better(o, c)) c = o;
                }
            }
            return block_argmax(c, red_key, red_pos, red_row, rb);
        };
        auto publish = [&](const Cand& mine, int jg, int jprev, const double* pw) {
            const unsigned epoch = (unsigned)(p.epoch_base + jg + 1);
            const int par = jg & 1;
            if constexpr (DSM) {
                const int words = 4 + 2 * nbc;
                for (int e = t; e < p.G * words; e += PT_THREADS) {
                    const int peer = e / words, w = e % words;
                    unsigned val;
                    const uint2* slot;
                    if (w < 4) {
                        val = w == 0 ? (unsigned)mine.key : w == 1 ? (unsigned)(mine.key >> 32) : w == 2 ? (unsigned)mine.pos : (unsigned)mine.row;
                        slot = cs_hdr + (size_t)(par * CS_MAX + cta) * 4 + w;
                    } else {
                        const int c = (w - 4) >> 1;
                        double x = 0.0;
                        if (mine.row >= 0) {
                            const int lrw = mine.row - row_base;
                            x = Ab[c * Rpad + lrw];
                            if (jprev >= 0 && c > jprev + 1) x = fma(-Ab[jprev * Rpad + lrw], pw[c], x);
                        }
                        const unsigned long long xb = (unsigned long long)__double_as_longlong(x);
                        val = ((w - 4) & 1) ? (unsigned)(xb >> 32) : (unsigned)xb;
                        slot = cs_row + (size_t)(par * CS_MAX + cta) * 2 * NB + (w - 4);
                    }
                    st_ll_dsmem(slot, (unsigned)peer, val, epoch);
                }
                return;
            }
            uint2* myhdr = p.slot_hdr + (size_t)(par * MAXG + cta) * 4;
            if (t < 4) {
                const unsigned w = t == 0 ? (unsigned)mine.key : t == 1 ? (unsigned)(mine.key >> 32)
                                 : t == 2 ? (unsigned)mine.pos : (unsigned)mine.row;
                st_ll(myhdr + t, w, epoch);
            }
            if (t < nbc) {
                double x = 0.0;
                if (mine.row >= 0) {
                    const int lrw = mine.row - row_base;
                    x = Ab[t * Rpad + lrw];
                    if (jprev >= 0 && t > jprev + 1) x = fma(-Ab[jprev * Rpad + lrw], pw[t], x);
                }
                const unsigned long long xb = (unsigned long long)__double_as_longlong(x);
                uint2* myrow = p.slot_rows + (size_t)(par * MAXG + cta) * 64 + 2 * t;
                st_ll(myrow, (unsigned)xb, epoch);
                st_ll(myrow + 1, (unsigned)(xb >> 32), epoch);
            }
        };
        {
            const Cand mine0 = local_candidate(0);
            TICK(0)
            if (t < 32) __threadfence();
            publish(mine0, jb, -1, nullptr);
        }
        for (int j = 0; j < nsb; ++j) {
            const int jg = jb + j;
            const int par = jg & 1;
            double* pr = prow + par * NB;
            {
                const unsigned epoch = (unsigned)(p.epoch_base + jg + 1);
                if (p.G > 32) {
                    Cand gc{0ull, INT_MAX, -1};
                    for (int g = t; g < p.G; g += PT_THREADS) {
                        const uint2* h = p.slot_hdr + (size_t)(par * MAXG + g) * 4;
                        uint4 a, b;
                        do {
                            a = ld_ll2(h);
                            b = ld_ll2(h + 2);
                        } while (a.y != epoch || a.w != epoch || b.y != epoch || b.w != epoch);
                        Cand o{((unsigned long long)a.z << 32) | a.x, (int)b.x, (int)b.z};
                        if (better(o, gc)) gc = o;
                    }
                    TICK(1)
                    const Cand w = block_argmax(gc, red_key, red_pos, red_row, rb);
                    TICK(2)
                    const int wcta = w.row / p.R;
                    if (t < nbc) {
                        const uint2* wr = p.slot_rows + (size_t)(par * MAXG + wcta) * 64 + 2 * t;
                        uint4 a;
                        do {
                            a = ld_ll2(wr);
                        } while (a.y != epoch || a.w != epoch);
                        const double x = __longlong_as_double((long long)(((unsigned long long)a.z << 32) | a.x));
                        pr[t] = x;
                        LU11[j * (NB + 1) + t] = x;
                    }
                    if (t == 0) {
                        win_sh[2 * par] = w.pos;
                        win_sh[2 * par + 1] = w.row;
                    }
                } else if (t < 32) {
                    Cand gc{0ull, INT_MAX, -1};
                    if (t < p.G) {
                        uint4 a, b;
                        if constexpr (DSM) {
                            const uint2* h = cs_hdr + (size_t)(par * CS_MAX + t) * 4;
                            do {
                                a = ld_ll2_smem(h);
                                b = ld_ll2_smem(h + 2);
                            } while (a.y != epoch || a.w != epoch || b.y != epoch || b.w != epoch);
                        } else {
                            const uint2* h = p.slot_hdr + (size_t)(par * MAXG + t) * 4;
                            do {
                                a = ld_ll2(h);
                                b = ld_ll2(h + 2);
                            } while (a.y != epoch || a.w != epoch || b.y != epoch || b.w != epoch);
                        }
                        gc = Cand{((unsigned long long)a.z << 32) | a.x, (int)b.x, (int)b.z};
                    }
                    TICK(1)
                    const Cand w = warp_argmax(gc);
                    TICK(2)
                    if ((DSM || !p.spec) && t < nbc) {
                        uint4 a;
                        if constexpr (DSM) {
                            const uint2* wr = cs_row + (size_t)(par * CS_MAX + w.row / p.R) * 2 * NB + 2 * t;
                            do {
                                a = ld_ll2_smem(wr);
                            } while (a.y != epoch || a.w != epoch);
                        } else {
                            const uint2* wr = p.slot_rows + (size_t)(par * MAXG + w.row / p.R) * 64 + 2 * t;
                            do {
                                a = ld_ll2(wr);
                            } while (a.y != epoch || a.w != epoch);
                        }
                        crow[(size_t)par * 32 * NB + (size_t)(w.row / p.R) * NB + t] =
                            __longlong_as_double((long long)(((unsigned long long)a.z << 32) | a.x));
                    }
                    if (t == 0) {
                        win_sh[2 * par] = w.pos;
                        win_sh[2 * par + 1] = w.row;
                    }
                } else if (!DSM && p.spec) {
                    double* cr = crow + (size_t)par * 32 * NB;
                    constexpr int SPEC_T = PT_THREADS - 32;
                    constexpr int SPEC_MAX = (32 * NB + SPEC_T - 1) / SPEC_T;
                    const int e0 = t - 32, tot = p.G * nbc;
                    uint4 a[SPEC_MAX];
                    unsigned pending = 0;
#pragma unroll
                    for (int i = 0; i < SPEC_MAX; ++i)
                        if (e0 + i * SPEC_T < tot) pending |= 1u << i;
                    while (pending) {
#pragma unroll
                        for (int i = 0; i < SPEC_MAX; ++i) {
                            if (pending & (1u << i)) {
                                const int e = e0 + i * SPEC_T;
                                a[i] = ld_ll2(p.slot_rows + (size_t)(par * MAXG + e / nbc) * 64 + 2 * (e % nbc));
                            }
                        }
#pragma unroll
                        for (int i = 0; i < SPEC_MAX; ++i) {
                            if ((pending & (1u << i)) && a[i].y == epoch && a[i].w == epoch) {
                                const int e = e0 + i * SPEC_T;
                                cr[(e / nbc) * NB + e % nbc] = __longlong_as_double((long long)(((unsigned long long)a[i].z << 32) | a[i].x));
                                pending &= ~(1u << i);
                            }
                        }
                    }
                }
            }
            __syncthreads();
            Cand win;
            win.key = 0;
            win.pos = win_sh[2 * par];
            win.row = win_sh[2 * par + 1];
            if (p.G <= 32) {
                pr = crow + (size_t)par * 32 * NB + (size_t)(win.row / p.R) * NB;
                if (t < nbc) LU11[j * (NB + 1) + t] = pr[t];
            }
            if (t == 0) {
                pivrow_blk[j] = win.row;
                if (cta == 0) p.perm_out[jg] = win.row;
            }
            TICK(3)
            const double pivot = pr[j];
            const double rinv = pivot != 0.0 ? 1.0 / pivot : 0.0;
            const bool have_next = (j + 1 < nbc);
            const double pnext = have_next ? pr[j + 1] : 0.0;
            double lq[RPT_MAX];
#pragma unroll
            for (int q = 0; q < RPT_MAX; ++q) {
                const int lr = t + q * PT_THREADS;
                lq[q] = 0.0;
                if (!active[q]) continue;
                if (row_base + lr == win.row) {
                    active[q] = false;
                    s_act[lr] = 0;
                    pib[q] = j;
                    continue;
                }
                if (pos[q] == jg) pos[q] = win.pos;
                if (pivot != 0.0) {
                    lq[q] = Ab[j * Rpad + lr] * rinv;
                    Ab[j * Rpad + lr] = lq[q];
                }
                if (have_next) Ab[(j + 1) * Rpad + lr] = fma(-lq[q], pnext, Ab[(j + 1) * Rpad + lr]);
            }
            if (j + 1 < nsb) {
                const Cand mine = local_candidate(j + 1);
                TICK(0)
                publish(mine, jg + 1, j, pr);
                __syncthreads();
            }
            {
                double* __restrict__ ab = Ab;
#pragma unroll 4
                for (int c2 = j + 2; c2 < nbc; ++c2) {
                    const double pc = pr[c2];
#pragma unroll
                    for (int q = 0; q < RPT_MAX; ++q) {
                        const int lr = t + q * PT_THREADS;
                        if (active[q]) ab[c2 * Rpad + lr] = fma(-lq[q], pc, ab[c2 * Rpad + lr]);
                    }
                }
            }
            TICK(4)
        }

        __syncthreads();
        for (int e = t; e < nbc * Rpad; e += PT_THREADS) {
            const int c = e / Rpad, lr = e - c * Rpad;
            if (lr < Rloc) W[(int64_t)(jb + c) * ldw + row_base + lr] = Ab[e];
        }
        if (cta == 0 && p.A00 != nullptr) {
            for (int e = t; e < nsb * nbc; e += PT_THREADS) {
                const int i = e / nbc, c = e % nbc;
                p.A00[(size_t)(jb + i) * v + jb + c] = LU11[i * (NB + 1) + c];
            }
        }

        TICK(5)
        const int cstart = jb + nbc;
        const int rem = v - cstart;
        if (rem > 0) {
            __syncthreads();
            __threadfence();
            for (int cc = t; cc < rem; cc += PT_THREADS) {
                const double* col = W + (int64_t)(cstart + cc) * ldw;
                double u[NB];
#pragma unroll
                for (int i = 0; i < NB; ++i) u[i] = (i < nsb) ? ld_cg_f64(col + pivrow_blk[i]) : 0.0;
#pragma unroll
                for (int i = 1; i < NB; ++i) {
                    if (i < nsb) {
#pragma unroll
                        for (int s2 = 0; s2 < i; ++s2) u[i] -= LU11[i * (NB + 1) + s2] * u[s2];
                    }
                }
#pragma unroll
                for (int i = 0; i < NB; ++i) U12[i * v + cc] = u[i];
                if (cta == 0 && p.A00 != nullptr) {
#pragma unroll
                    for (int i = 0; i < NB; ++i)
                        if (i < nsb) p.A00[(size_t)(jb + i) * v + cstart + cc] = u[i];
                }
            }
            __syncthreads();
            TICK(6)
            auto update_row = [&](int lr, int cfirst, int cstep, bool tail) {
                double l[NB];
#pragma unroll
                for (int i = 0; i < NB; ++i) l[i] = (i < nsb) ? Ab[i * Rpad + lr] : 0.0;
                double* wp = W + (int64_t)cstart * ldw + row_base + lr;
                int cc = cfirst;
                double w0 = 0, w1 = 0, w2 = 0, w3 = 0;
                if (cc + 3 < rem) {
                    w0 = wp[(int64_t)cc * ldw];
                    w1 = wp[(int64_t)(cc + 1) * ldw];
                    w2 = wp[(int64_t)(cc + 2) * ldw];
                    w3 = wp[(int64_t)(cc + 3) * ldw];
                }
                for (; cc + 3 < rem; cc += cstep) {
                    double n0 = 0, n1 = 0, n2 = 0, n3 = 0;
                    const int cn = cc + cstep;
                    if (cn + 3 < rem) {
                        n0 = wp[(int64_t)cn * ldw];
                        n1 = wp[(int64_t)(cn + 1) * ldw];
                        n2 = wp[(int64_t)(cn + 2) * ldw];
                        n3 = wp[(int64_t)(cn + 3) * ldw];
                    }
#pragma unroll
                    for (int i = 0; i < NB; ++i) {
                        const double2 ua = *reinterpret_cast<const double2*>(U12 + i * v + cc);
                        const double2 ub = *reinterpret_cast<const double2*>(U12 + i * v + cc + 2);
                        w0 -= l[i] * ua.x;
                        w1 -= l[i] * ua.y;
                        w2 -= l[i] * ub.x;
                        w3 -= l[i] * ub.y;
                    }
                    wp[(int64_t)cc * ldw] = w0;
                    wp[(int64_t)(cc + 1) * ldw] = w1;
                    wp[(int64_t)(cc + 2) * ldw] = w2;
                    wp[(int64_t)(cc + 3) * ldw] = w3;
                    w0 = n0;
                    w1 = n1;
                    w2 = n2;
                    w3 = n3;
                }
                if (tail) {
                    for (int ct = rem & ~3; ct < rem; ++ct) {
                        double x = wp[(int64_t)ct * ldw];
#pragma unroll
                        for (int i = 0; i < NB; ++i) x -= l[i] * U12[i * v + ct];
                        wp[(int64_t)ct * ldw] = x;
                    }
                }
            };
            if (RPT_MAX == 1 && p.R < PT_THREADS) {
                const int nshare = PT_THREADS / p.R;
                const int lr = t % p.R, part = t / p.R;
                if (part < nshare && lr < Rloc && s_act[lr]) update_row(lr, 4 * part, 4 * nshare, part == 0);
            } else {
#pragma unroll 1
                for (int q = 0; q < RPT_MAX; ++q) {
                    const int lr = t + q * PT_THREADS;
                    if (lr >= Rloc || !active[q]) continue;
                    update_row(lr, 0, 4, true);
                }
            }
        }
#pragma unroll
        for (int q = 0; q < RPT_MAX; ++q) pib[q] = -1;
        __threadfence();
        __syncthreads();
        TICK(7)
    }
    if (cta == 0)
        for (int i = p.nsteps + t; i < v; i += PT_THREADS) p.perm_out[i] = i;
    if (cta == 0 && t == 0 && p.dbg != nullptr)
        for (int i = 0; i < 8; ++i) p.dbg[i] = tm[i];
    if constexpr (DSM) cluster_sync_all();
#undef TICK
}

constexpr int SK_CB = 16;
struct StackArgs {
    double* W;
    int64_t ldw;
    int n, v;
    int* perm_out;
    int* ppos;
    unsigned* flags;
    unsigned* ticket;
    unsigned ticket_base, epoch;
};
__device__ __forceinline__ unsigned ld_acquire_u32(const unsigned* p) {
    unsigned v;
    asm volatile("ld.acquire.gpu.global.u32 %0, [%1];" : "=r"(v) : "l"(p) : "memory");
    return v;
}
__device__ __forceinline__ void st_release_u32(unsigned* p, unsigned v) {
    asm volatile("st.release.gpu.global.u32 [%0], %1;" ::"l"(p), "r"(v) : "memory");
}
__device__ __forceinline__ void cp_async16(double* smem_dst, const double* gsrc) {
    asm volatile("cp.async.cg.shared.global [%0], [%1], 16;" ::"r"(smem_u32(smem_dst)), "l"(gsrc) : "memory");
}
__device__ __forceinline__ void cp_async_commit() { asm volatile("cp.async.commit_group;" ::: "memory"); }
__device__ __forceinline__ void cp_async_wait_all() { asm volatile("cp.async.wait_all;" ::: "memory"); }

template <int NT>
__global__ void __launch_bounds__(NT, 1) stack_getrf_kernel(StackArgs p) {
    __shared__ double A12s[SK_CB][SK_CB + 1];
    __shared__ double L11s[SK_CB][SK_CB + 1];
    __shared__ double prow[2][SK_CB];
    __shared__ unsigned long long red_key[2][32];
    __shared__ int red_pos[2][32], red_row[2][32];
    __shared__ int pivs[SK_CB], ppos_s[SK_CB];
    __shared__ int s_cta;
    extern __shared__ __align__(16) double Ls[];
    const int t = threadIdx.x, warp = t >> 5, lane = t & 31, nw = blockDim.x >> 5;
    if (t == 0) s_cta = (int)(atomicAdd(p.ticket, 1u) - p.ticket_base);
    __syncthreads();
    const int c = s_cta, c0 = c * SK_CB;
    const bool valid = t < p.n;
    double* __restrict__ W = p.W;
    const int64_t ldw = p.ldw;
    double a[SK_CB];
#pragma unroll
    for (int j = 0; j < SK_CB; ++j) a[j] = valid ? W[(int64_t)(c0 + j) * ldw + t] : 0.0;
    int pos = t;
    int mypiv = -1;

    for (int b = 0; b < c; ++b) {
        if (t == 0)
            while (ld_acquire_u32(p.flags + b) != p.epoch) {}
        __syncthreads();
        if (t < SK_CB) {
            pivs[t] = ld_cg_s32(p.perm_out + b * SK_CB + t);
            ppos_s[t] = ld_cg_s32(p.ppos + b * SK_CB + t);
        }
        {
            const int half = blockDim.x >> 1, q = t % half, h = t / half;
            if (2 * q < p.n) {
                const double* lp = W + (int64_t)(b * SK_CB + 8 * h) * ldw + 2 * q;
#pragma unroll
                for (int k = 0; k < SK_CB / 2; ++k) cp_async16(Ls + (8 * h + k) * NT + 2 * q, lp + (int64_t)k * ldw);
            }
        }
        cp_async_commit();
        __syncthreads();
        int kk = -1;
        if (mypiv < 0) {
#pragma unroll
            for (int k = 0; k < SK_CB; ++k) {
                if (pivs[k] == t) kk = k;
                else if (kk < 0 && pos == b * SK_CB + k) pos = ppos_s[k];
            }
        }
        if (kk >= 0) {
#pragma unroll
            for (int j = 0; j < SK_CB; ++j) A12s[kk][j] = a[j];
#pragma unroll
            for (int k = 0; k < SK_CB; ++k) L11s[kk][k] = ld_cg_f64(W + (int64_t)(b * SK_CB + k) * ldw + t);
        }
        __syncthreads();
        if (t < SK_CB) {
#pragma unroll
            for (int i = 1; i < SK_CB; ++i) {
                double x = A12s[i][t];
#pragma unroll
                for (int s2 = 0; s2 < i; ++s2) x = fma(-L11s[i][s2], A12s[s2][t], x);
                A12s[i][t] = x;
            }
        }
        cp_async_wait_all();
        __syncthreads();
        if (kk >= 0) {
#pragma unroll
            for (int j = 0; j < SK_CB; ++j) a[j] = A12s[kk][j];
            mypiv = b * SK_CB + kk;
        } else if (mypiv < 0 && valid) {
#pragma unroll
            for (int k = 0; k < SK_CB; ++k) {
                const double lk = Ls[k * NT + t];
#pragma unroll
                for (int j = 0; j < SK_CB; ++j) a[j] = fma(-lk, A12s[k][j], a[j]);
            }
        }
    }

#pragma unroll
    for (int j = 0; j < SK_CB; ++j) {
        const int jg = c0 + j, par = j & 1;
        Cand cd{0ull, INT_MAX, -1};
        if (valid && mypiv < 0) cd = Cand{(unsigned long long)__double_as_longlong(fabs(a[j])), pos, t};
        const Cand w1 = warp_argmax(cd);
        if (lane == 0) {
            red_key[par][warp] = w1.key;
            red_pos[par][warp] = w1.pos;
            red_row[par][warp] = w1.row;
        }
        __syncthreads();
        Cand x{0ull, INT_MAX, -1};
        if (lane < nw) x = Cand{red_key[par][lane], red_pos[par][lane], red_row[par][lane]};
        const Cand win = warp_argmax(x);
        if (t == win.row) {
#pragma unroll
            for (int m = 0; m < SK_CB; ++m) prow[par][m] = a[m];
            mypiv = jg;
        }
        if (t == 0) {
            p.perm_out[jg] = win.row;
            p.ppos[jg] = win.pos;
        }
        __syncthreads();
        if (valid && mypiv < 0) {
            if (pos == jg) pos = win.pos;
            const double pivot = prow[par][j];
            const double rinv = pivot != 0.0 ? 1.0 / pivot : 0.0;
            double lq = 0.0;
            if (pivot != 0.0) {
                lq = a[j] * rinv;
                a[j] = lq;
            }
#pragma unroll
            for (int m = j + 1; m < SK_CB; ++m) a[m] = fma(-lq, prow[par][m], a[m]);
        }
    }
    if (valid) {
#pragma unroll
        for (int j = 0; j < SK_CB; ++j) W[(int64_t)(c0 + j) * ldw + t] = a[j];
    }
    __threadfence();
    __syncthreads();
    if (t == 0) st_release_u32(p.flags + c, p.epoch);
}

int launch_stack_getrf(double* W, int64_t ldw, int n, int v, int* perm_out, PanelWorkspace* ws, cudaStream_t stream) {
    StackArgs a{};
    a.W = W;
    a.ldw = ldw;
    a.n = n;
    a.v = v;
    a.perm_out = perm_out;
    a.ppos = ws->sk_ppos;
    a.flags = ws->sk_flags;
    a.ticket = ws->sk_ticket;
    a.ticket_base = ws->sk_ticket_count;
    a.epoch = ++ws->sk_epoch;
    const int C = v / SK_CB;
    ws->sk_ticket_count += (unsigned)C;
    const int threads = (int)round_up(n, 32);
    static PerDeviceMax cfg;
    if (cfg.raise((size_t)SK_CB * 1024 * sizeof(double))) {
        CFLX_CUDA(cudaFuncSetAttribute(stack_getrf_kernel<1024>, cudaFuncAttributeMaxDynamicSharedMemorySize, SK_CB * 1024 * 8));
        CFLX_CUDA(cudaFuncSetAttribute(stack_getrf_kernel<512>, cudaFuncAttributeMaxDynamicSharedMemorySize, SK_CB * 512 * 8));
    }
    if (threads <= 256) stack_getrf_kernel<256><<<C, threads, SK_CB * 256 * sizeof(double), stream>>>(a);
    else if (threads <= 512) stack_getrf_kernel<512><<<C, threads, SK_CB * 512 * sizeof(double), stream>>>(a);
    else stack_getrf_kernel<1024><<<C, threads, SK_CB * 1024 * sizeof(double), stream>>>(a);
    CFLX_CUDA(cudaGetLastError());
    return CFLX_OK;
}

template <int NB>
size_t panel_smem_bytes(int Rpad, int v) {
    return ((size_t)NB * Rpad + (size_t)NB * v + NB * (NB + 1) + 2 * NB + 2 * 32 * NB) * sizeof(double) +
           2 * PT_WARPS * (sizeof(unsigned long long) + 2 * sizeof(int)) + (NB + 4) * sizeof(int) +
           2 * CS_MAX * (4 + 2 * NB) * sizeof(uint2) + (size_t)Rpad + 64;
}

template <int NB, int RPT>
int launch_nb_rpt(PanelArgs& a, bool cluster, cudaStream_t stream) {
    const size_t smem = panel_smem_bytes<NB>(a.Rpad, a.v);
    void* params[] = {&a};
    if (cluster) {
        static PerDeviceMax cfg;
        if (cfg.raise(smem))
            CFLX_CUDA(cudaFuncSetAttribute(panel_getrf_kernel<NB, RPT, true>, cudaFuncAttributeMaxDynamicSharedMemorySize, (int)smem));
        cudaLaunchConfig_t lc{};
        lc.gridDim = dim3(a.G);
        lc.blockDim = dim3(PT_THREADS);
        lc.dynamicSmemBytes = smem;
        lc.stream = stream;
        cudaLaunchAttribute at[1];
        at[0].id = cudaLaunchAttributeClusterDimension;
        at[0].val.clusterDim.x = a.G;
        at[0].val.clusterDim.y = 1;
        at[0].val.clusterDim.z = 1;
        lc.attrs = at;
        lc.numAttrs = 1;
        CFLX_CUDA(cudaLaunchKernelExC(&lc, (const void*)panel_getrf_kernel<NB, RPT, true>, params));
        return CFLX_OK;
    }
    static PerDeviceMax cfg;
    if (cfg.raise(smem))
        CFLX_CUDA(cudaFuncSetAttribute(panel_getrf_kernel<NB, RPT, false>, cudaFuncAttributeMaxDynamicSharedMemorySize, (int)smem));
    CFLX_CUDA(cudaLaunchCooperativeKernel((void*)panel_getrf_kernel<NB, RPT, false>, dim3(a.G), dim3(PT_THREADS), params, smem, stream));
    return CFLX_OK;
}
template <int NB>
int launch_nb(PanelArgs& a, bool cluster, cudaStream_t stream) {
    const int rpt = (a.R + PT_THREADS - 1) / PT_THREADS;
    if (rpt <= 1) return launch_nb_rpt<NB, 1>(a, cluster, stream);
    if (rpt <= 2) return launch_nb_rpt<NB, 2>(a, cluster, stream);
    if (rpt <= 4) return launch_nb_rpt<NB, 4>(a, cluster, stream);
    return launch_nb_rpt<NB, 8>(a, cluster, stream);
}
}

int panel_workspace_create(PanelWorkspace* ws) {
    int dev = 0, sms = 0;
    CFLX_CUDA(cudaGetDevice(&dev));
    CFLX_CUDA(cudaDeviceGetAttribute(&sms, cudaDevAttrMultiProcessorCount, dev));
    ws->max_ctas = sms < MAXG ? sms : MAXG;
    ws->epoch = 1;
    ws->cta_cap = 0;
    CFLX_CUDA(cudaMalloc(&ws->slot_hdr, sizeof(uint2) * 2 * MAXG * 4));
    CFLX_CUDA(cudaMalloc(&ws->slot_rows, sizeof(uint2) * 2 * MAXG * 64));
    CFLX_CUDA(cudaMalloc(&ws->dbg, sizeof(long long) * 8));
    CFLX_CUDA(cudaMemset(ws->dbg, 0, sizeof(long long) * 8));
    CFLX_CUDA(cudaMemset(ws->slot_hdr, 0, sizeof(uint2) * 2 * MAXG * 4));
    CFLX_CUDA(cudaMemset(ws->slot_rows, 0, sizeof(uint2) * 2 * MAXG * 64));
    CFLX_CUDA(cudaMalloc(&ws->sk_flags, sizeof(unsigned) * 1024));
    CFLX_CUDA(cudaMalloc(&ws->sk_ppos, sizeof(int) * 16384));
    CFLX_CUDA(cudaMalloc(&ws->sk_ticket, sizeof(unsigned)));
    CFLX_CUDA(cudaMemset(ws->sk_flags, 0, sizeof(unsigned) * 1024));
    CFLX_CUDA(cudaMemset(ws->sk_ticket, 0, sizeof(unsigned)));
    ws->sk_epoch = 0;
    ws->sk_ticket_count = 0;
    {
        const char* e = getenv("CFLX_STACK_KERNEL");
        ws->sk_enabled = e ? atoi(e) : 1;
    }
    return CFLX_OK;
}
void panel_workspace_destroy(PanelWorkspace* ws) {
    cudaFree(ws->slot_hdr);
    cudaFree(ws->dbg);
    cudaFree(ws->slot_rows);
    cudaFree(ws->sk_flags);
    cudaFree(ws->sk_ppos);
    cudaFree(ws->sk_ticket);
    *ws = PanelWorkspace{};
}

int launch_panel_getrf_a00(double* W, int64_t ldw, int n, int v, int* perm_out, double* A00, int* nb_used,
                           PanelWorkspace* ws, cudaStream_t stream) {
    if (v <= 0 || n < 0) return CFLX_ERR_ARG;
    if (ws->sk_enabled && n >= v && n <= 1024 && v % SK_CB == 0 && v <= 16384 && ldw % 2 == 0 &&
        (reinterpret_cast<uintptr_t>(W) & 15) == 0) {
        if (nb_used) *nb_used = 0;
        return launch_stack_getrf(W, ldw, n, v, perm_out, ws, stream);
    }
    PanelArgs a{};
    a.W = W;
    a.ldw = ldw;
    a.n = n;
    a.v = v;
    a.nsteps = n < v ? n : v;
    static int cluster_rows = -1;
    if (cluster_rows < 0) {
        const char* e = getenv("CFLX_CLUSTER_ROWS");
        cluster_rows = e ? atoi(e) : 0;
    }
    const bool cluster = n > 0 && n <= cluster_rows;
    int G = (n + 31) / 32;
    if (G < 1) G = 1;
    if (G > ws->max_ctas) G = ws->max_ctas;
    if (ws->cta_cap > 0 && G > ws->cta_cap) {
        G = ws->cta_cap;
        const int need = (n + RPT_LIMIT * PT_THREADS - 1) / (RPT_LIMIT * PT_THREADS);
        if (G < need) G = need < ws->max_ctas ? need : ws->max_ctas;
    }
    if (cluster && G > CS_MAX) G = CS_MAX;
    int R = (n + G - 1) / G;
    R = (int)round_up(R > 0 ? R : 1, 32);
    G = n > 0 ? (n + R - 1) / R : 1;
    if (R > RPT_LIMIT * PT_THREADS) {
        set_last_error("panel_getrf: n=%d rows exceed the %d-row capacity (%d CTAs x %d rows)", n,
                       ws->max_ctas * RPT_LIMIT * PT_THREADS, ws->max_ctas, RPT_LIMIT * PT_THREADS);
        return CFLX_ERR_UNSUPPORTED;
    }
    a.R = R;
    a.Rpad = R;
    a.G = G;
    a.perm_out = perm_out;
    a.A00 = A00;
    a.slot_hdr = reinterpret_cast<uint2*>(ws->slot_hdr);
    a.slot_rows = reinterpret_cast<uint2*>(ws->slot_rows);
    a.epoch_base = ws->epoch;
    {
        static int spec = -1;
        if (spec < 0) {
            const char* e = getenv("CFLX_PANEL_SPEC");
            spec = e ? atoi(e) : 0;
        }
        a.spec = spec;
    }
    a.dbg = ws->dbg;
    ws->epoch += v + 2 + (v & 1);
    const size_t budget = 222 * 1024;
    int nb = v >= 32 ? 32 : (v >= 16 ? 16 : (v >= 8 ? 8 : 4));
    if (nb == 32 && panel_smem_bytes<32>(a.Rpad, v) > budget) nb = 16;
    if (nb == 16 && panel_smem_bytes<16>(a.Rpad, v) > budget) nb = 8;
    if (nb == 8 && panel_smem_bytes<8>(a.Rpad, v) > budget) nb = 4;
    if (nb == 4 && panel_smem_bytes<4>(a.Rpad, v) > budget) {
        set_last_error("panel_getrf: v=%d with %d rows per CTA needs %zu B of shared memory (budget %zu)", v, a.Rpad,
                       panel_smem_bytes<4>(a.Rpad, v), budget);
        return CFLX_ERR_UNSUPPORTED;
    }
    if (nb_used) *nb_used = nb;
    switch (nb) {
        case 32: return launch_nb<32>(a, cluster, stream);
        case 16: return launch_nb<16>(a, cluster, stream);
        case 8: return launch_nb<8>(a, cluster, stream);
        default: return launch_nb<4>(a, cluster, stream);
    }
}

int launch_panel_getrf(double* W, int64_t ldw, int n, int v, int* perm_out, PanelWorkspace* ws, cudaStream_t stream) {
    return launch_panel_getrf_a00(W, ldw, n, v, perm_out, nullptr, nullptr, ws, stream);
}

}
```

### include/conflux_b200.h

```cpp
#ifndef CONFLUX_B200_H
#define CONFLUX_B200_H

#include <stddef.h>
#include <stdint.h>

#ifdef __cplusplus
extern "C" {
#endif

typedef enum {
    CFLX_OK = 0,
    CFLX_ERR_ARG = -1,
    CFLX_ERR_CUDA = -2,
    CFLX_ERR_NCCL = -3,
    CFLX_ERR_UNSUPPORTED = -4,
    CFLX_ERR_STATE = -5,
    CFLX_ERR_NO_DEVICE = -6
} cflx_status;

typedef struct cflx_comm cflx_comm;
typedef struct cflx_lu cflx_lu;

#define CFLX_UNIQUE_ID_BYTES 128

const char* cflx_last_error(void);
const char* cflx_version(void);
int cflx_device_count(int* count);

int cflx_get_unique_id(void* id_out );
int cflx_comm_create(int world_size, int world_rank, const void* unique_id, int device, cflx_comm** out);
int cflx_comm_barrier(cflx_comm*);
void cflx_comm_destroy(cflx_comm*);

int cflx_host_alloc(size_t bytes, void** out);
int cflx_host_free(void* p);

int cflx_auto_grid(int M, int N, int P, int* Px, int* Py, int* Pz);
int cflx_lu_dims(int M, int N, int v, int Px, int Py, int Pz, int* dims_out);
int cflx_init_matrix_host(int M, int N, int v, int Px, int Py, int Pz, int rank, int seed, double* local_out);

int cflx_lu_create(cflx_comm*, int M, int N, int v, int Px, int Py, int Pz, cflx_lu** out);
int cflx_lu_info(const cflx_lu*, int* info_out);
int cflx_lu_set_local(cflx_lu*, const double* host_local);
int cflx_lu_queue_next_local(cflx_lu*, const double* host_next);
int cflx_lu_factor(cflx_lu*, double* ms_out);
int cflx_lu_get_factors(cflx_lu*, double* C_host, int* permutation_out);
int cflx_lu_get_permutation(cflx_lu*, int* permutation_out);
int cflx_lu_validate(cflx_lu*, double* frob_abs_out, double* frob_rel_out);
int cflx_lu_residual(cflx_lu*, double* rel_out);
int cflx_lu_solve(cflx_lu*, int nrhs, const double* B_local, double* X_local, double* ms_out);
int cflx_lu_uses_tcgen05(const cflx_lu*);
int cflx_lu_launch_count(cflx_lu*, int64_t* count_out, int reset);
int cflx_lu_set_profiling(cflx_lu*, int mode);
int cflx_lu_phase_ms(cflx_lu*, double* ms_out);
int cflx_lu_timeline(cflx_lu*, char* buf, int buf_len);
int cflx_lu_set_kernel_timing(cflx_lu*, int enabled);
int cflx_lu_trailing_stats(cflx_lu*, double* ms_out, double* flops_out);
void cflx_lu_destroy(cflx_lu*);

typedef struct cflx_chol cflx_chol;
int cflx_chol_auto_grid(int P, int N, int* grid3_out);
int cflx_chol_auto_tile(int N, int P, int Pz);
int cflx_chol_dims(int N, int v, int Px, int Py, int Pz, int* dims_out);
int cflx_chol_init_matrix_host(int N, int v, int Px, int Py, int Pz, int rank, double* local_out);
int cflx_chol_create(cflx_comm*, int N, int v, int Px, int Py, int Pz, cflx_chol** out);
int cflx_chol_info(const cflx_chol*, int* info_out);
int cflx_chol_set_local(cflx_chol*, const double* host_local);
int cflx_chol_factor(cflx_chol*, double* ms_out);
int cflx_chol_get_local(cflx_chol*, double* L_host);
int cflx_chol_validate(cflx_chol*, double* frob_abs_out, double* frob_rel_out);
int cflx_chol_launch_count(cflx_chol*, int64_t* count_out, int reset);
void cflx_chol_destroy(cflx_chol*);

int cflx_dbg_gemm_tn(int M, int N, int K, const double* AT, const double* B, const double* C, double alpha, double beta,
                     double* D, int reps, double* ms_out);
int cflx_dbg_panel(int n, int v, const double* panel, int* perm_out, double* A00_out, double* LU_out, int reps,
                   double* ms_out);
int cflx_dbg_trsm(int n, int v, const double* A00, const double* B, double* X_out, const double* R, double* Y_out);
int cflx_dbg_trsm_left_upper(int v, int n, const double* A00, const double* R, double* X_out);
int cflx_dbg_potrf_tile(int v, int blocked, const double* A, double* L_out, double* LT_out, int* info_out);
int cflx_dbg_ozaki_gemm(int M, int N, int K, const double* AT, const double* B, const double* C, double* D,
                        signed char* planesA_out, signed char* planesB_out, int* ea_out, int* eb_out, int reps,
                        double* ms_out, double* split_ms_out);
int cflx_dbg_umma_peak(int which, int n, double* tmacs_out);
int cflx_dbg_push_pivots(int n_rows, int n_cols, double* A_inout, int npiv, const int* pivot_rows, int fnpr, int* gri_out,
                         double* a01_out);
int cflx_dbg_last_panel_cycles(long long* out8);
int cflx_dbg_fp64_peak(int which, double* tflops_out);
int cflx_dbg_fp64_peak_ex(int which, double* burst_out, double* sustained_out);

#ifdef __cplusplus
}
#endif
#endif
```

Measured before the change: 30000.

## Enable 16-CTA cluster panel factorization with DSMEM pivot exchange and stream gate

Panel LU now runs by default as a 16-CTA thread-block cluster for mid-size panels (1024 < n <= 16K rows). Each CTA writes its pivot candidate and row into its own shared memory, and peers read them over distributed shared memory behind cluster barriers, replacing the epoch-polled global slots and extra threadfences. A global gate word, written once the cluster starts, is waited on with cuStreamWaitValue32 so the trailing GEMM on the main stream leaves only 16 SMs free for the panel instead of the full CTA cap. The risks are cluster scheduling limits, the fixed 16-CTA row partition, and the extra cross-stream wait.

```diff
diff --git a/conflux_b200/_lib.py b/conflux_b200/_lib.py
--- a/conflux_b200/_lib.py
+++ b/conflux_b200/_lib.py
@@ -20,7 +20,7 @@
     "cflx_lu_get_permutation", "cflx_lu_residual", "cflx_lu_validate", "cflx_lu_solve", "cflx_lu_launch_count", "cflx_lu_uses_tcgen05", "cflx_lu_set_profiling", "cflx_lu_phase_ms", "cflx_lu_timeline",
     "cflx_lu_set_kernel_timing", "cflx_lu_trailing_stats", "cflx_lu_destroy", "cflx_chol_auto_grid", "cflx_chol_auto_tile", "cflx_chol_dims", "cflx_chol_init_matrix_host",
     "cflx_chol_create", "cflx_chol_info", "cflx_chol_set_local", "cflx_chol_factor", "cflx_chol_get_local", "cflx_chol_validate",
-    "cflx_chol_launch_count", "cflx_chol_destroy", "cflx_dbg_gemm_tn", "cflx_dbg_panel", "cflx_dbg_trsm", "cflx_dbg_trsm_left_upper", "cflx_dbg_potrf_tile", "cflx_dbg_push_pivots", "cflx_dbg_ozaki_gemm", "cflx_dbg_umma_peak", "cflx_dbg_last_panel_cycles", "cflx_dbg_fp64_peak", "cflx_dbg_fp64_peak_ex",
+    "cflx_chol_launch_count", "cflx_chol_destroy", "cflx_dbg_gemm_tn", "cflx_dbg_panel", "cflx_dbg_trsm", "cflx_dbg_trsm_left_upper", "cflx_dbg_potrf_tile", "cflx_dbg_push_pivots", "cflx_dbg_ozaki_gemm", "cflx_dbg_umma_peak", "cflx_dbg_last_panel_cycles", "cflx_dbg_last_panel_kernel", "cflx_dbg_fp64_peak", "cflx_dbg_fp64_peak_ex",
 ]
 
 
diff --git a/conflux_b200/csrc/dbg.cu b/conflux_b200/csrc/dbg.cu
--- a/conflux_b200/csrc/dbg.cu
+++ b/conflux_b200/csrc/dbg.cu
@@ -58,11 +58,17 @@
 }
 
 static long long g_panel_cycles[8] = {0};
+static int g_panel_kernel = -1;
 
 extern "C" {
 
 int cflx_dbg_last_panel_cycles(long long* out8) {
     for (int i = 0; i < 8; ++i) out8[i] = g_panel_cycles[i];
+    return CFLX_OK;
+}
+
+int cflx_dbg_last_panel_kernel(int* kind_out) {
+    *kind_out = g_panel_kernel;
     return CFLX_OK;
 }
 
@@ -186,6 +192,7 @@
     if (rc == CFLX_OK && n >= v)
         rc = launch_gather_a00(dW.as<double>(), ld, dperm.as<int>(), v, nb, dA00.as<double>(), dA00T.as<double>(), 0);
     cudaMemcpy(g_panel_cycles, ws.dbg, sizeof(g_panel_cycles), cudaMemcpyDeviceToHost);
+    g_panel_kernel = ws.last_kernel;
     panel_workspace_destroy(&ws);
     if (rc != CFLX_OK) {
         if (rc == CFLX_ERR_CUDA) set_last_error("panel kernel failed: %s", cudaGetErrorString(cudaGetLastError()));
diff --git a/conflux_b200/csrc/kernels.h b/conflux_b200/csrc/kernels.h
--- a/conflux_b200/csrc/kernels.h
+++ b/conflux_b200/csrc/kernels.h
@@ -37,6 +37,7 @@
 int umma_peak_probe(int n, int use_f16, double* tmacs_out);
 int launch_ozaki_gemm(OzakiWorkspace* ws, int M, int N, int row0, int col0, double* C, int64_t ldc, int max_ctas, cudaStream_t s);
 
+constexpr int PANEL_CLUSTER_CTAS = 16;
 struct PanelWorkspace {
     void* slot_hdr;
     void* slot_rows;
@@ -49,6 +50,11 @@
     unsigned* sk_ticket;
     unsigned sk_epoch, sk_ticket_count;
     int sk_enabled;
+    int cluster_ok;
+    unsigned* gate;
+    unsigned gate_seq;
+    unsigned gate_first;
+    int last_kernel;
 };
 int panel_workspace_create(PanelWorkspace* ws);
 void panel_workspace_destroy(PanelWorkspace* ws);
diff --git a/conflux_b200/csrc/lu.cu b/conflux_b200/csrc/lu.cu
--- a/conflux_b200/csrc/lu.cu
+++ b/conflux_b200/csrc/lu.cu
@@ -423,6 +423,7 @@
             CFLX_CUDA(cudaEventRecord(lu->ev_fork, s));
             CFLX_CUDA(cudaStreamWaitEvent(sp, lu->ev_fork, 0));
         }
+        lu->pws.gate_first = 0;
         CFLX_TRY(panel_phase(lu, k + 1, fnpr, sp));
         if (side) CFLX_CUDA(cudaEventRecord(lu->ev_join, sp));
         if (split_u) {
@@ -432,7 +433,13 @@
         }
         if (split_u) CFLX_TRY(store_factors());
         if (split_u && n_act > 0) CFLX_TRY(ozaki_planes_b(lu, w, ncols - w, ldu, s));
-        const int leave = (side && lu->use_ozaki) ? lu->pws.cta_cap : 0;
+        const bool gate = side && lu->pws.gate_first != 0 && lu->stream_wait_value32 != nullptr;
+        if (gate && lu->stream_wait_value32((CUstream)s, (CUdeviceptr)lu->pws.gate, lu->pws.gate_first,
+                                            CU_STREAM_WAIT_VALUE_GEQ) != CUDA_SUCCESS) {
+            set_last_error("step %d: cuStreamWaitValue32 on the pivot-search gate failed", k);
+            return CFLX_ERR_CUDA;
+        }
+        const int leave = (side && lu->use_ozaki) ? (gate ? PANEL_CLUSTER_CTAS : lu->pws.cta_cap) : 0;
         CFLX_TRY(trailing_gemm(lu, k, 1, fnpr, n_act, c0 + w, ncols - w, ld2, ldu, w, s, leave > 0 ? lu->oz.sms - leave : 0));
         if (side) CFLX_CUDA(cudaStreamWaitEvent(s, lu->ev_join, 0));
     } else {
@@ -694,6 +701,15 @@
             if (cudaEventCreateWithFlags(&lu->ev_join, cudaEventDisableTiming) != cudaSuccess) return fail(CFLX_ERR_CUDA);
             const char* c = getenv("CFLX_PANEL_CTAS");
             lu->pws.cta_cap = c ? atoi(c) : (lu->P == 1 ? 32 : (lu->Px == 1 ? 48 : 64));
+            void* fn = nullptr;
+            cudaDriverEntryPointQueryResult q{};
+            if (cudaGetDriverEntryPoint("cuStreamWaitValue32", &fn, cudaEnableDefault, &q) == cudaSuccess &&
+                q == cudaDriverEntryPointSuccess)
+                lu->stream_wait_value32 = reinterpret_cast<decltype(lu->stream_wait_value32)>(fn);
+            else {
+                cudaGetLastError();
+                lu->pws.cluster_ok = 0;
+            }
         }
     }
     cudaMemsetAsync(lu->PT, 0, pan * sizeof(double), c->stream);
diff --git a/conflux_b200/csrc/lu_state.h b/conflux_b200/csrc/lu_state.h
--- a/conflux_b200/csrc/lu_state.h
+++ b/conflux_b200/csrc/lu_state.h
@@ -1,4 +1,5 @@
 #pragma once
+#include <cuda.h>
 #include <nccl.h>
 
 #include <algorithm>
@@ -104,6 +105,7 @@
     std::vector<char> ev_used;
     cudaStream_t side = nullptr;
     cudaEvent_t ev_fork = nullptr, ev_join = nullptr, ev_npiv = nullptr;
+    CUresult (*stream_wait_value32)(CUstream, CUdeviceptr, cuuint32_t, unsigned int) = nullptr;
     cflx::SolveState sv;
 };
 
diff --git a/conflux_b200/csrc/panel.cu b/conflux_b200/csrc/panel.cu
--- a/conflux_b200/csrc/panel.cu
+++ b/conflux_b200/csrc/panel.cu
@@ -26,6 +26,8 @@
     int epoch_base;
     int spec;
     long long* dbg;
+    unsigned* gate;
+    unsigned gate_seq;
 };
 
 __device__ __forceinline__ void st_ll(uint2* p, unsigned data, unsigned epoch) {
@@ -37,21 +39,25 @@
     return v;
 }
 
-constexpr int CS_MAX = 8;
-__device__ __forceinline__ void st_ll_dsmem(const uint2* local_slot, unsigned peer, unsigned data, unsigned epoch) {
+constexpr int CL_CTAS = PANEL_CLUSTER_CTAS;
+__device__ __forceinline__ unsigned dsmem_addr(const void* local, unsigned peer) {
     unsigned remote;
-    asm volatile("mapa.shared::cluster.u32 %0, %1, %2;" : "=r"(remote) : "r"(smem_u32(local_slot)), "r"(peer));
-    asm volatile("st.shared::cluster.v2.u32 [%0], {%1, %2};" ::"r"(remote), "r"(data), "r"(epoch) : "memory");
-}
-__device__ __forceinline__ uint4 ld_ll2_smem(const uint2* p) {
+    asm volatile("mapa.shared::cluster.u32 %0, %1, %2;" : "=r"(remote) : "r"(smem_u32(local)), "r"(peer));
+    return remote;
+}
+__device__ __forceinline__ uint4 ld_dsmem_v4(const void* local, unsigned peer) {
     uint4 v;
-    asm volatile("ld.volatile.shared.v4.u32 {%0, %1, %2, %3}, [%4];" : "=r"(v.x), "=r"(v.y), "=r"(v.z), "=r"(v.w) : "r"(smem_u32(p)) : "memory");
+    asm volatile("ld.shared::cluster.v4.u32 {%0, %1, %2, %3}, [%4];" : "=r"(v.x), "=r"(v.y), "=r"(v.z), "=r"(v.w)
+                 : "r"(dsmem_addr(local, peer)) : "memory");
     return v;
 }
-__device__ __forceinline__ void cluster_sync_all() {
-    asm volatile("barrier.cluster.arrive.release.aligned;" ::: "memory");
-    asm volatile("barrier.cluster.wait.acquire.aligned;" ::: "memory");
-}
+__device__ __forceinline__ double ld_dsmem_f64(const double* local, unsigned peer) {
+    double v;
+    asm volatile("ld.shared::cluster.f64 %0, [%1];" : "=d"(v) : "r"(dsmem_addr(local, peer)) : "memory");
+    return v;
+}
+__device__ __forceinline__ void cluster_arrive() { asm volatile("barrier.cluster.arrive.release.aligned;" ::: "memory"); }
+__device__ __forceinline__ void cluster_wait() { asm volatile("barrier.cluster.wait.acquire.aligned;" ::: "memory"); }
 
 struct Cand {
     unsigned long long key;
@@ -105,14 +111,14 @@
     double* LU11 = U12 + (size_t)NB * p.v;
     double* prow = LU11 + NB * (NB + 1);
     double* crow = prow + 2 * NB;
-    unsigned long long* red_key = reinterpret_cast<unsigned long long*>(crow + 2 * 32 * NB);
+    double* cl_row = crow + 2 * 32 * NB;
+    uint4* cl_hdr = reinterpret_cast<uint4*>(cl_row + 2 * NB);
+    unsigned long long* red_key = reinterpret_cast<unsigned long long*>(cl_hdr + 2);
     int* red_pos = reinterpret_cast<int*>(red_key + 2 * PT_WARPS);
     int* red_row = red_pos + 2 * PT_WARPS;
     int* pivrow_blk = red_row + 2 * PT_WARPS;
     int* win_sh = pivrow_blk + NB;
-    uint2* cs_hdr = reinterpret_cast<uint2*>(win_sh + 4);
-    uint2* cs_row = cs_hdr + 2 * CS_MAX * 4;
-    unsigned char* s_act = reinterpret_cast<unsigned char*>(cs_row + 2 * CS_MAX * 2 * NB);
+    unsigned char* s_act = reinterpret_cast<unsigned char*>(win_sh + 4);
     int rb = 0;
 
     const int t = threadIdx.x;
@@ -140,11 +146,8 @@
         pib[q] = -1;
     }
     for (int lr = t; lr < Rpad; lr += PT_THREADS) s_act[lr] = lr < Rloc ? 1 : 0;
-    if constexpr (DSM) {
-        for (int e = t; e < 2 * CS_MAX * (4 + 2 * NB); e += PT_THREADS) cs_hdr[e] = make_uint2(0u, 0u);
-        __syncthreads();
-        cluster_sync_all();
-    }
+    if (DSM && cta == 0 && t == 0 && p.gate != nullptr)
+        asm volatile("st.release.sys.global.u32 [%0], %1;" ::"l"(p.gate), "r"(p.gate_seq) : "memory");
 
     for (int jb = 0; jb < p.nsteps; jb += NB) {
         const int nbc = min(NB, v - jb);
@@ -172,27 +175,16 @@
             const unsigned epoch = (unsigned)(p.epoch_base + jg + 1);
             const int par = jg & 1;
             if constexpr (DSM) {
-                const int words = 4 + 2 * nbc;
-                for (int e = t; e < p.G * words; e += PT_THREADS) {
-                    const int peer = e / words, w = e % words;
-                    unsigned val;
-                    const uint2* slot;
-                    if (w < 4) {
-                        val = w == 0 ? (unsigned)mine.key : w == 1 ? (unsigned)(mine.key >> 32) : w == 2 ? (unsigned)mine.pos : (unsigned)mine.row;
-                        slot = cs_hdr + (size_t)(par * CS_MAX + cta) * 4 + w;
-                    } else {
-                        const int c = (w - 4) >> 1;
-                        double x = 0.0;
-                        if (mine.row >= 0) {
-                            const int lrw = mine.row - row_base;
-                            x = Ab[c * Rpad + lrw];
-                            if (jprev >= 0 && c > jprev + 1) x = fma(-Ab[jprev * Rpad + lrw], pw[c], x);
-                        }
-                        const unsigned long long xb = (unsigned long long)__double_as_longlong(x);
-                        val = ((w - 4) & 1) ? (unsigned)(xb >> 32) : (unsigned)xb;
-                        slot = cs_row + (size_t)(par * CS_MAX + cta) * 2 * NB + (w - 4);
-                    }
-                    st_ll_dsmem(slot, (unsigned)peer, val, epoch);
+                if (t == 0)
+                    cl_hdr[par] = make_uint4((unsigned)mine.key, (unsigned)(mine.key >> 32), (unsigned)mine.pos, (unsigned)mine.row);
+                if (t < nbc) {
+                    double x = 0.0;
+                    if (mine.row >= 0) {
+                        const int lrw = mine.row - row_base;
+                        x = Ab[t * Rpad + lrw];
+                        if (jprev >= 0 && t > jprev + 1) x = fma(-Ab[jprev * Rpad + lrw], pw[t], x);
+                    }
+                    cl_row[par * NB + t] = x;
                 }
                 return;
             }
@@ -218,8 +210,12 @@
         {
             const Cand mine0 = local_candidate(0);
             TICK(0)
-            if (t < 32) __threadfence();
+            if (!DSM && t < 32) __threadfence();
             publish(mine0, jb, -1, nullptr);
+            if constexpr (DSM) {
+                __syncthreads();
+                cluster_arrive();
+            }
         }
         for (int j = 0; j < nsb; ++j) {
             const int jg = jb + j;
@@ -227,7 +223,38 @@
             double* pr = prow + par * NB;
             {
                 const unsigned epoch = (unsigned)(p.epoch_base + jg + 1);
-                if (p.G > 32) {
+                if constexpr (DSM) {
+                    cluster_wait();
+                    if (t < 32) {
+                        Cand gc{0ull, INT_MAX, -1};
+                        if (t < p.G) {
+                            const uint4 h = ld_dsmem_v4(cl_hdr + par, (unsigned)t);
+                            gc = Cand{((unsigned long long)h.y << 32) | h.x, (int)h.z, (int)h.w};
+                        }
+                        TICK(1)
+                        const Cand w = warp_argmax(gc);
+                        TICK(2)
+                        if (t == 0) {
+                            win_sh[2 * par] = w.pos;
+                            win_sh[2 * par + 1] = w.row;
+                        }
+                    } else {
+                        constexpr int ROW_T = PT_THREADS - 32;
+                        constexpr int ROW_MAX = (CL_CTAS * NB + ROW_T - 1) / ROW_T;
+                        const int e0 = t - 32, tot = p.G * nbc;
+                        double x[ROW_MAX];
+#pragma unroll
+                        for (int i = 0; i < ROW_MAX; ++i) {
+                            const int e = e0 + i * ROW_T;
+                            if (e < tot) x[i] = ld_dsmem_f64(cl_row + par * NB + e % nbc, (unsigned)(e / nbc));
+                        }
+#pragma unroll
+                        for (int i = 0; i < ROW_MAX; ++i) {
+                            const int e = e0 + i * ROW_T;
+                            if (e < tot) crow[(size_t)par * 32 * NB + (e / nbc) * NB + e % nbc] = x[i];
+                        }
+                    }
+                } else if (p.G > 32) {
                     Cand gc{0ull, INT_MAX, -1};
                     for (int g = t; g < p.G; g += PT_THREADS) {
                         const uint2* h = p.slot_hdr + (size_t)(par * MAXG + g) * 4;
@@ -261,37 +288,22 @@
                     Cand gc{0ull, INT_MAX, -1};
                     if (t < p.G) {
                         uint4 a, b;
-                        if constexpr (DSM) {
-                            const uint2* h = cs_hdr + (size_t)(par * CS_MAX + t) * 4;
-                            do {
-                                a = ld_ll2_smem(h);
-                                b = ld_ll2_smem(h + 2);
-                            } while (a.y != epoch || a.w != epoch || b.y != epoch || b.w != epoch);
-                        } else {
-                            const uint2* h = p.slot_hdr + (size_t)(par * MAXG + t) * 4;
-                            do {
-                                a = ld_ll2(h);
-                                b = ld_ll2(h + 2);
-                            } while (a.y != epoch || a.w != epoch || b.y != epoch || b.w != epoch);
-                        }
+                        const uint2* h = p.slot_hdr + (size_t)(par * MAXG + t) * 4;
+                        do {
+                            a = ld_ll2(h);
+                            b = ld_ll2(h + 2);
+                        } while (a.y != epoch || a.w != epoch || b.y != epoch || b.w != epoch);
                         gc = Cand{((unsigned long long)a.z << 32) | a.x, (int)b.x, (int)b.z};
                     }
                     TICK(1)
                     const Cand w = warp_argmax(gc);
                     TICK(2)
-                    if ((DSM || !p.spec) && t < nbc) {
+                    if (!p.spec && t < nbc) {
                         uint4 a;
-                        if constexpr (DSM) {
-                            const uint2* wr = cs_row + (size_t)(par * CS_MAX + w.row / p.R) * 2 * NB + 2 * t;
-                            do {
-                                a = ld_ll2_smem(wr);
-                            } while (a.y != epoch || a.w != epoch);
-                        } else {
-                            const uint2* wr = p.slot_rows + (size_t)(par * MAXG + w.row / p.R) * 64 + 2 * t;
-                            do {
-                                a = ld_ll2(wr);
-                            } while (a.y != epoch || a.w != epoch);
-                        }
+                        const uint2* wr = p.slot_rows + (size_t)(par * MAXG + w.row / p.R) * 64 + 2 * t;
+                        do {
+                            a = ld_ll2(wr);
+                        } while (a.y != epoch || a.w != epoch);
                         crow[(size_t)par * 32 * NB + (size_t)(w.row / p.R) * NB + t] =
                             __longlong_as_double((long long)(((unsigned long long)a.z << 32) | a.x));
                     }
@@ -299,7 +311,7 @@
                         win_sh[2 * par] = w.pos;
                         win_sh[2 * par + 1] = w.row;
                     }
-                } else if (!DSM && p.spec) {
+                } else if (p.spec) {
                     double* cr = crow + (size_t)par * 32 * NB;
                     constexpr int SPEC_T = PT_THREADS - 32;
                     constexpr int SPEC_MAX = (32 * NB + SPEC_T - 1) / SPEC_T;
@@ -370,6 +382,7 @@
                 TICK(0)
                 publish(mine, jg + 1, j, pr);
                 __syncthreads();
+                if constexpr (DSM) cluster_arrive();
             }
             {
                 double* __restrict__ ab = Ab;
@@ -403,7 +416,7 @@
         const int rem = v - cstart;
         if (rem > 0) {
             __syncthreads();
-            __threadfence();
+            if (!DSM) __threadfence();
             for (int cc = t; cc < rem; cc += PT_THREADS) {
                 const double* col = W + (int64_t)(cstart + cc) * ldw;
                 double u[NB];
@@ -490,7 +503,7 @@
         }
 #pragma unroll
         for (int q = 0; q < RPT_MAX; ++q) pib[q] = -1;
-        __threadfence();
+        if (!DSM) __threadfence();
         __syncthreads();
         TICK(7)
     }
@@ -498,7 +511,10 @@
         for (int i = p.nsteps + t; i < v; i += PT_THREADS) p.perm_out[i] = i;
     if (cta == 0 && t == 0 && p.dbg != nullptr)
         for (int i = 0; i < 8; ++i) p.dbg[i] = tm[i];
-    if constexpr (DSM) cluster_sync_all();
+    if constexpr (DSM) {
+        cluster_arrive();
+        cluster_wait();
+    }
 #undef TICK
 }
 
@@ -684,19 +700,30 @@
 
 template <int NB>
 size_t panel_smem_bytes(int Rpad, int v) {
-    return ((size_t)NB * Rpad + (size_t)NB * v + NB * (NB + 1) + 2 * NB + 2 * 32 * NB) * sizeof(double) +
-           2 * PT_WARPS * (sizeof(unsigned long long) + 2 * sizeof(int)) + (NB + 4) * sizeof(int) +
-           2 * CS_MAX * (4 + 2 * NB) * sizeof(uint2) + (size_t)Rpad + 64;
-}
+    return ((size_t)NB * Rpad + (size_t)NB * v + NB * (NB + 1) + 2 * NB + 2 * 32 * NB + 2 * NB) * sizeof(double) +
+           2 * sizeof(uint4) + 2 * PT_WARPS * (sizeof(unsigned long long) + 2 * sizeof(int)) + (NB + 4) * sizeof(int) +
+           (size_t)Rpad + 64;
+}
+
+constexpr size_t PANEL_SMEM_BUDGET = 222 * 1024;
 
 template <int NB, int RPT>
-int launch_nb_rpt(PanelArgs& a, bool cluster, cudaStream_t stream) {
+int cluster_func_attributes() {
+    static PerDeviceMax cfg;
+    if (cfg.raise(PANEL_SMEM_BUDGET)) {
+        CFLX_CUDA(cudaFuncSetAttribute(panel_getrf_kernel<NB, RPT, true>, cudaFuncAttributeMaxDynamicSharedMemorySize,
+                                       (int)PANEL_SMEM_BUDGET));
+        CFLX_CUDA(cudaFuncSetAttribute(panel_getrf_kernel<NB, RPT, true>, cudaFuncAttributeNonPortableClusterSizeAllowed, 1));
+    }
+    return CFLX_OK;
+}
+
+template <int NB, int RPT>
+int launch_nb_rpt(PanelArgs& a, bool cluster, PanelWorkspace* ws, cudaStream_t stream) {
     const size_t smem = panel_smem_bytes<NB>(a.Rpad, a.v);
     void* params[] = {&a};
     if (cluster) {
-        static PerDeviceMax cfg;
-        if (cfg.raise(smem))
-            CFLX_CUDA(cudaFuncSetAttribute(panel_getrf_kernel<NB, RPT, true>, cudaFuncAttributeMaxDynamicSharedMemorySize, (int)smem));
+        CFLX_TRY((cluster_func_attributes<NB, RPT>()));
         cudaLaunchConfig_t lc{};
         lc.gridDim = dim3(a.G);
         lc.blockDim = dim3(PT_THREADS);
@@ -710,6 +737,7 @@
         lc.attrs = at;
         lc.numAttrs = 1;
         CFLX_CUDA(cudaLaunchKernelExC(&lc, (const void*)panel_getrf_kernel<NB, RPT, true>, params));
+        if (ws->gate_first == 0) ws->gate_first = a.gate_seq;
         return CFLX_OK;
     }
     static PerDeviceMax cfg;
@@ -719,12 +747,12 @@
     return CFLX_OK;
 }
 template <int NB>
-int launch_nb(PanelArgs& a, bool cluster, cudaStream_t stream) {
+int launch_nb(PanelArgs& a, bool cluster, PanelWorkspace* ws, cudaStream_t stream) {
     const int rpt = (a.R + PT_THREADS - 1) / PT_THREADS;
-    if (rpt <= 1) return launch_nb_rpt<NB, 1>(a, cluster, stream);
-    if (rpt <= 2) return launch_nb_rpt<NB, 2>(a, cluster, stream);
-    if (rpt <= 4) return launch_nb_rpt<NB, 4>(a, cluster, stream);
-    return launch_nb_rpt<NB, 8>(a, cluster, stream);
+    if (rpt <= 1) return launch_nb_rpt<NB, 1>(a, cluster, ws, stream);
+    if (rpt <= 2) return launch_nb_rpt<NB, 2>(a, cluster, ws, stream);
+    if (rpt <= 4) return launch_nb_rpt<NB, 4>(a, cluster, ws, stream);
+    return launch_nb_rpt<NB, 8>(a, cluster, ws, stream);
 }
 }
 
@@ -752,6 +780,31 @@
         const char* e = getenv("CFLX_STACK_KERNEL");
         ws->sk_enabled = e ? atoi(e) : 1;
     }
+    CFLX_CUDA(cudaMalloc(&ws->gate, sizeof(unsigned)));
+    CFLX_CUDA(cudaMemset(ws->gate, 0, sizeof(unsigned)));
+    ws->gate_seq = 0;
+    ws->gate_first = 0;
+    ws->cluster_ok = 0;
+    const char* e = getenv("CFLX_CLUSTER_PANEL");
+    if (!e || atoi(e) != 0) {
+        CFLX_TRY((cluster_func_attributes<16, 4>()));
+        cudaLaunchConfig_t lc{};
+        lc.gridDim = dim3(CL_CTAS);
+        lc.blockDim = dim3(PT_THREADS);
+        lc.dynamicSmemBytes = PANEL_SMEM_BUDGET;
+        cudaLaunchAttribute at[1];
+        at[0].id = cudaLaunchAttributeClusterDimension;
+        at[0].val.clusterDim.x = CL_CTAS;
+        at[0].val.clusterDim.y = 1;
+        at[0].val.clusterDim.z = 1;
+        lc.attrs = at;
+        lc.numAttrs = 1;
+        int nclusters = 0;
+        if (cudaOccupancyMaxActiveClusters(&nclusters, (const void*)panel_getrf_kernel<16, 4, true>, &lc) == cudaSuccess)
+            ws->cluster_ok = nclusters > 0;
+        else
+            cudaGetLastError();
+    }
     return CFLX_OK;
 }
 void panel_workspace_destroy(PanelWorkspace* ws) {
@@ -761,6 +814,7 @@
     cudaFree(ws->sk_flags);
     cudaFree(ws->sk_ppos);
     cudaFree(ws->sk_ticket);
+    cudaFree(ws->gate);
     *ws = PanelWorkspace{};
 }
 
@@ -770,6 +824,7 @@
     if (ws->sk_enabled && n >= v && n <= 1024 && v % SK_CB == 0 && v <= 16384 && ldw % 2 == 0 &&
         (reinterpret_cast<uintptr_t>(W) & 15) == 0) {
         if (nb_used) *nb_used = 0;
+        ws->last_kernel = 0;
         return launch_stack_getrf(W, ldw, n, v, perm_out, ws, stream);
     }
     PanelArgs a{};
@@ -778,12 +833,7 @@
     a.n = n;
     a.v = v;
     a.nsteps = n < v ? n : v;
-    static int cluster_rows = -1;
-    if (cluster_rows < 0) {
-        const char* e = getenv("CFLX_CLUSTER_ROWS");
-        cluster_rows = e ? atoi(e) : 0;
-    }
-    const bool cluster = n > 0 && n <= cluster_rows;
+    const bool cluster = ws->cluster_ok && n > 1024 && n <= CL_CTAS * 1024;
     int G = (n + 31) / 32;
     if (G < 1) G = 1;
     if (G > ws->max_ctas) G = ws->max_ctas;
@@ -792,10 +842,10 @@
         const int need = (n + RPT_LIMIT * PT_THREADS - 1) / (RPT_LIMIT * PT_THREADS);
         if (G < need) G = need < ws->max_ctas ? need : ws->max_ctas;
     }
-    if (cluster && G > CS_MAX) G = CS_MAX;
+    if (cluster) G = CL_CTAS;
     int R = (n + G - 1) / G;
     R = (int)round_up(R > 0 ? R : 1, 32);
-    G = n > 0 ? (n + R - 1) / R : 1;
+    if (!cluster) G = n > 0 ? (n + R - 1) / R : 1;
     if (R > RPT_LIMIT * PT_THREADS) {
         set_last_error("panel_getrf: n=%d rows exceed the %d-row capacity (%d CTAs x %d rows)", n,
                        ws->max_ctas * RPT_LIMIT * PT_THREADS, ws->max_ctas, RPT_LIMIT * PT_THREADS);
@@ -818,8 +868,12 @@
         a.spec = spec;
     }
     a.dbg = ws->dbg;
+    if (cluster) {
+        a.gate = ws->gate;
+        a.gate_seq = ++ws->gate_seq;
+    }
     ws->epoch += v + 2 + (v & 1);
-    const size_t budget = 222 * 1024;
+    const size_t budget = PANEL_SMEM_BUDGET;
     int nb = v >= 32 ? 32 : (v >= 16 ? 16 : (v >= 8 ? 8 : 4));
     if (nb == 32 && panel_smem_bytes<32>(a.Rpad, v) > budget) nb = 16;
     if (nb == 16 && panel_smem_bytes<16>(a.Rpad, v) > budget) nb = 8;
@@ -830,11 +884,12 @@
         return CFLX_ERR_UNSUPPORTED;
     }
     if (nb_used) *nb_used = nb;
+    ws->last_kernel = cluster ? 2 : 1;
     switch (nb) {
-        case 32: return launch_nb<32>(a, cluster, stream);
-        case 16: return launch_nb<16>(a, cluster, stream);
-        case 8: return launch_nb<8>(a, cluster, stream);
-        default: return launch_nb<4>(a, cluster, stream);
+        case 32: return launch_nb<32>(a, cluster, ws, stream);
+        case 16: return launch_nb<16>(a, cluster, ws, stream);
+        case 8: return launch_nb<8>(a, cluster, ws, stream);
+        default: return launch_nb<4>(a, cluster, ws, stream);
     }
 }
 
diff --git a/include/conflux_b200.h b/include/conflux_b200.h
--- a/include/conflux_b200.h
+++ b/include/conflux_b200.h
@@ -86,6 +86,7 @@
 int cflx_dbg_push_pivots(int n_rows, int n_cols, double* A_inout, int npiv, const int* pivot_rows, int fnpr, int* gri_out,
                          double* a01_out);
 int cflx_dbg_last_panel_cycles(long long* out8);
+int cflx_dbg_last_panel_kernel(int* kind_out);
 int cflx_dbg_fp64_peak(int which, double* tflops_out);
 int cflx_dbg_fp64_peak_ex(int which, double* burst_out, double* sustained_out);
 
```

Measured after the change: 24570 (median of 6 runs). -18.1%, worse.
